# gisbi-kim/lt-mapper

Hardware: AMD Instinct MI355X
Metric: keyframe-pairs/sec (removert+diff) (higher is better)
Workload: dtype f32; 1 GPU; lot-2x500-os1-64-3res; sensor=os1-64

## Files before the change

### include/ltm.h

```cpp
#ifndef LTM_H
#define LTM_H

#include <stddef.h>
#include <stdint.h>

#ifdef __cplusplus
extern "C" {
#endif

#define LTM_ABI_VERSION 1

enum {
    LTM_OK = 0,
    LTM_E_INVALID = -1,
    LTM_E_DEVICE = -2,
    LTM_E_NOMEM = -3,
    LTM_E_UNSUPPORTED = -4
};

typedef struct ltm_ctx ltm_ctx;
typedef uint64_t ltm_cloud;
typedef uint64_t ltm_scanset;
typedef uint64_t ltm_poses;

// ... 36 lines not shown
int ltm_scanset_concat(ltm_ctx*, const ltm_scanset* in, size_t n, ltm_scanset* out);
int ltm_scanset_zip_concat(ltm_ctx*, ltm_scanset a, ltm_scanset b, ltm_scanset c, ltm_scanset* out);
int ltm_scanset_alloc(ltm_ctx*, const uint64_t* offsets, size_t n_kf, ltm_scanset* out);
int ltm_scanset_free(ltm_ctx*, ltm_scanset);

int ltm_buffer_alloc(ltm_ctx*, size_t bytes, void** dev);
int ltm_buffer_free(ltm_ctx*, void* dev);
int ltm_buffer_fill(ltm_ctx*, void* dev, int byte_value, size_t bytes);
int ltm_buffer_copy(ltm_ctx*, void* dst, const void* src, size_t bytes, int kind);

typedef uint64_t ltm_upload;
int ltm_scanset_upload_begin(ltm_ctx*, size_t capacity_points, ltm_upload* up);
int ltm_scanset_upload_chunk(ltm_ctx*, ltm_upload up, const void* pts, size_t stride_bytes, const uint64_t* kf_sizes, size_t n_kf);
int ltm_scanset_upload_end(ltm_ctx*, ltm_upload up, ltm_scanset* out);

typedef struct ltm_fetch ltm_fetch;
int ltm_cloud_fetch_begin(ltm_ctx*, ltm_cloud, ltm_fetch** out);
int ltm_scanset_fetch_begin(ltm_ctx*, ltm_scanset, ltm_fetch** out);
int ltm_fetch_wait(ltm_fetch*, const void** host_xyzi, size_t* n_points, const uint64_t** offsets, size_t* n_kf);
int ltm_fetch_release(ltm_ctx*, ltm_fetch*);
int ltm_cloud_fetch_chunks_begin(ltm_ctx*, ltm_cloud, ltm_fetch** out);
int ltm_scanset_fetch_chunks_begin(ltm_ctx*, ltm_scanset, ltm_fetch** out);
int ltm_fetch_info(ltm_fetch*, size_t* n_points, const uint64_t** offsets, size_t* n_kf);
int ltm_fetch_next_chunk(ltm_fetch*, const void** host_xyzi, size_t* first_point, size_t* n_points, size_t* first_kf, size_t* n_kf);
int ltm_fetch_chunk_done(ltm_fetch*, const void* host_xyzi);

int ltm_poses_create(ltm_ctx*, size_t n_kf, const double* poses, const double* inv_or_null, ltm_poses* out);
int ltm_inverse4x4(const double* m16, double* inv16);
int ltm_poses_free(ltm_ctx*, ltm_poses);


int ltm_preclean(ltm_ctx*, ltm_scanset in, float radius, ltm_scanset* out);

int ltm_merge_to_global(ltm_ctx*, ltm_scanset scans, ltm_poses poses, ltm_cloud* out);

int ltm_voxel_centroid(ltm_ctx*, ltm_cloud in, float leaf, ltm_cloud* out);
int ltm_voxel_centroid_batch(ltm_ctx*, size_t n, const ltm_cloud* in, const float* leaf, ltm_cloud* out);
int ltm_voxel_centroid_shard(ltm_ctx*, ltm_cloud in, float leaf, uint32_t shard, uint32_t n_shards, ltm_cloud* out);
int ltm_cloud_bbox(ltm_ctx*, ltm_cloud in, float mn[3], float mx[3]);
int ltm_voxel_key_histogram(ltm_ctx*, ltm_cloud in, const float mn[3], const float mx[3], float leaf, uint32_t hist[4096]);
int ltm_voxel_key_split(ltm_ctx*, ltm_cloud in, const float mn[3], const float mx[3], float leaf, uint32_t n_parts, const uint32_t* cut_bins, ltm_cloud* parts);
int ltm_voxel_centroid_box(ltm_ctx*, ltm_cloud in, const float mn[3], const float mx[3], float leaf, ltm_cloud* out);
int ltm_voxel_centroid_scanset(ltm_ctx*, ltm_scanset in, float leaf, ltm_scanset* out);

int ltm_voxel_grid_scanset(ltm_ctx*, ltm_scanset in, float leaf, ltm_scanset* out);
typedef struct ltm_vgs ltm_vgs;
int ltm_voxel_grid_scanset_begin(ltm_ctx*, ltm_scanset in, float leaf, ltm_vgs** ticket);
int ltm_voxel_grid_scanset_end(ltm_ctx*, ltm_vgs* ticket, ltm_scanset* out);

int ltm_visibility_vote(ltm_ctx*, ltm_cloud map, ltm_scanset scans, ltm_poses poses, size_t kf_begin, size_t kf_end,
                        float res_alpha, float diff_thres, int mode, uint8_t* labels_dev);
int ltm_scanset_prepare_range_images(ltm_ctx*, ltm_scanset scans, size_t kf_begin, size_t kf_end, const float* res_alphas, size_t n_alphas);
int ltm_partition_by_labels(ltm_ctx*, ltm_cloud map, const uint8_t* labels_dev, ltm_cloud* kept, ltm_cloud* flagged);
int ltm_visibility_partition(ltm_ctx*, ltm_cloud map, ltm_scanset scans, ltm_poses poses, float res_alpha,
                             float diff_thres, int mode, ltm_cloud* kept, ltm_cloud* flagged, uint8_t* host_labels);

int ltm_reproject(ltm_ctx*, ltm_cloud map, ltm_poses poses, size_t kf_begin, size_t kf_end, float res_alpha, ltm_scanset* out);

int ltm_knn_partition(ltm_ctx*, ltm_cloud target, ltm_scanset scans, ltm_poses poses, size_t kf_begin, size_t kf_end,
                      int k, float thr, ltm_scanset* coexist, ltm_scanset* diff);
int ltm_knn_split_cloud(ltm_ctx*, ltm_cloud target, ltm_cloud query, int k, float thr, ltm_cloud* near, ltm_cloud* far);

typedef struct ltm_search ltm_search;
typedef struct ltm_search_result ltm_search_result;
int ltm_search_build(ltm_ctx*, ltm_cloud target, ltm_search** out);
int ltm_search_free(ltm_ctx*, ltm_search*);
int ltm_search_info(ltm_ctx*, ltm_search*, size_t* n_target, size_t* n_finite);
int ltm_knn_search(ltm_ctx*, ltm_search*, ltm_cloud query, int k, int32_t* idx_dev, float* d2_dev);
int ltm_radius_search(ltm_ctx*, ltm_search*, ltm_cloud query, float radius, int max_nn, ltm_search_result** out);
int ltm_search_result_info(ltm_ctx*, ltm_search_result*, size_t* n_query, size_t* total,
                           const uint64_t** offsets_dev, const int32_t** idx_dev, const float** d2_dev);
int ltm_search_result_free(ltm_ctx*, ltm_search_result*);

int ltm_search_estimate_normals(ltm_ctx*, size_t n_idx, ltm_search* const* idx, int k,
                                const float* viewpoints3_or_null );
int ltm_search_normals_info(ltm_ctx*, ltm_search*, int* k , const void** normals_dev );
int ltm_search_normals_download(ltm_ctx*, ltm_search*, float* nxyzc_host );

typedef struct ltm_sc ltm_sc;
typedef struct {
    double lidar_height;
    int    num_ring;
    int    num_sector;
    double max_radius;
    int    num_candidates;
    double search_ratio;
    double dist_thres;
} ltm_sc_params;
void ltm_sc_default_params(ltm_sc_params*);
int  ltm_sc_from_scanset(ltm_ctx*, ltm_scanset, size_t kf_begin, size_t kf_end, const ltm_sc_params*, ltm_sc** out);
int  ltm_sc_from_descriptors(ltm_ctx*, const double* desc_host, size_t n, const ltm_sc_params*, ltm_sc** out);
int  ltm_sc_info(ltm_ctx*, ltm_sc*, size_t* n, int* num_ring, int* num_sector);
int  ltm_sc_download(ltm_ctx*, ltm_sc*, double* desc, float* ring_keys, double* sector_keys);
int  ltm_sc_distance(ltm_ctx*, ltm_sc* a, ltm_sc* b, const int32_t* pairs_host, size_t n_pairs, const ltm_sc_params*, double* dist_host, int32_t* shift_host);
int  ltm_sc_detect(ltm_ctx*, ltm_sc* database, ltm_sc* queries, const ltm_sc_params*, int32_t* loop_id, int32_t* nn_idx, double* min_dist, int32_t* nn_align,
                   float* yaw_diff_rad);
int  ltm_sc_free(ltm_ctx*, ltm_sc*);

typedef struct {
    double max_corr_dist;
    int    max_iterations;
    double transformation_epsilon;
    double euclidean_fitness_epsilon;
} ltm_icp_params;
typedef struct {
    double   T[16];
    double   fitness;
    double   last_mse;
    int32_t  converged;
    int32_t  iterations;
    int32_t  state;
    uint32_t n_corr;
} ltm_icp_result;
void ltm_icp_default_params(ltm_icp_params*);
int  ltm_icp_align(ltm_ctx*, size_t n_pairs, ltm_search* const* targets, const ltm_cloud* sources,
                   const double* init16_or_null , const ltm_icp_params*,
                   ltm_icp_result* results_host, double* trace_host_or_null );
int  ltm_icp_align_scanset(ltm_ctx*, size_t n_pairs, ltm_search* const* targets, ltm_scanset sources, const uint32_t* source_kf ,
                           const double* init16_or_null, const ltm_icp_params*, ltm_icp_result* results_host, double* trace_host_or_null);

int  ltm_icp_align_plane(ltm_ctx*, size_t n_pairs, ltm_search* const* targets, const ltm_cloud* sources,
                         const double* init16_or_null, const ltm_icp_params*, ltm_icp_result* results_host, double* trace_host_or_null);
int  ltm_icp_align_plane_scanset(ltm_ctx*, size_t n_pairs, ltm_search* const* targets, ltm_scanset sources, const uint32_t* source_kf ,
                                 const double* init16_or_null, const ltm_icp_params*, ltm_icp_result* results_host, double* trace_host_or_null);

int ltm_pose6d_to_affine3f(const float* xyzrpy , size_t n, float* affine12 );
int ltm_submaps_assemble(ltm_ctx*, ltm_scanset scans, const float* affine12_host_or_null ,
                         const int32_t* keys_host, size_t n_windows, int search_num, float leaf, int order, ltm_scanset* out);
int ltm_search_build_scanset(ltm_ctx*, ltm_scanset, size_t kf_begin, size_t kf_end, ltm_search** out );

typedef struct ltm_event ltm_event;
int  ltm_lane_create(ltm_ctx* parent, ltm_ctx** lane);
int  ltm_lane_fence(ltm_ctx* done_in, ltm_ctx* before_next_of);
int  ltm_event_record(ltm_ctx*, ltm_event** ev);
int  ltm_event_wait(ltm_ctx*, ltm_event* ev);
void ltm_event_destroy(ltm_event* ev);
int  ltm_cloud_lend(ltm_ctx* from, ltm_cloud h, ltm_ctx* to, ltm_cloud* out);
int  ltm_cloud_give(ltm_ctx* from, ltm_cloud h, ltm_ctx* to, ltm_cloud* out);
int  ltm_scanset_lend(ltm_ctx* from, ltm_scanset h, ltm_ctx* to, ltm_scanset* out);
int  ltm_scanset_give(ltm_ctx* from, ltm_scanset h, ltm_ctx* to, ltm_scanset* out);
int ltm_debug_range_image(ltm_ctx*, ltm_cloud pts, const double* T1, const double* T2, float res_alpha,
                          float* rimg, int32_t* ptidx);
int ltm_debug_viz_images(ltm_ctx*, ltm_cloud map, ltm_scanset scans, ltm_poses poses, size_t kf, float res_alpha, int mode,
                         float range_min, float range_max, float diff_min, float diff_max,
                         uint8_t* scan_bgr, uint8_t* map_bgr, uint8_t* diff_bgr, uint8_t* ptidx_bgr);
int ltm_debug_project(ltm_ctx*, const float* xyz, size_t n, float res_alpha, float* out_az_el_r, int32_t* out_row_col);
void ltm_rimg_size(float vfov, float hfov, float res_alpha, int* rows, int* cols);
int ltm_debug_selfcheck(ltm_ctx*, uint64_t* mismatches3, int* fast_math_enabled);
int ltm_debug_elevation_fit(float vfov_deg, float* c4, double* max_err_rad);
int ltm_debug_pcl_sort_order(const uint32_t* leaf_idx, size_t n, uint32_t* order_out, int use_std_sort, uint32_t* heap_sort_fallbacks );
int ltm_debug_voxel_key_bits(const float* mn3, const float* mx3, float leaf, uint64_t* kept_mask, unsigned* depth, double* frame_min3);
int ltm_debug_proj_launch(float vfov, float hfov, float res_alpha, const double* base2lidar16_or_null, size_t map_points, size_t n_keyframes, int on_device,
                          float* out_f32, uint32_t* out_u32, uint32_t first_block, size_t n_blocks, uint32_t* out_tile, uint32_t* out_kf);
int ltm_debug_cull_check(ltm_ctx*, const float* xyz, size_t n, const double* inv_pose16_or_null, float res_alpha, uint64_t* violations);
int ltm_debug_cull_validation(ltm_ctx*, uint64_t* shapes_checked, uint64_t* shapes_failed);
int ltm_debug_occlusion_stats(ltm_ctx*, uint64_t* pairs, uint64_t* first_shell, uint64_t* projected, int reset);
int ltm_debug_voxel_stats(ltm_ctx*, uint64_t* grids, uint64_t* identity_hits, int reset);
int ltm_debug_knn_stats(ltm_ctx*, uint64_t* queries, uint64_t* undecided, uint64_t* two_phase_calls, uint64_t* unsorted_queue_calls, int reset);
int ltm_debug_sc_paths(int num_ring, int num_sector, int* scatter_in_lds, int* pair_in_lds);
int ltm_debug_cull_stats(ltm_ctx*, uint64_t* survivors, uint64_t* points, int reset);
int ltm_debug_pool_live(ltm_ctx*, uint64_t* live_blocks, uint64_t* live_bytes);

int ltm_profile_enable(ltm_ctx*, int on);
int ltm_profile_reset(ltm_ctx*);
int ltm_profile_read(ltm_ctx*, const char** names, double* ms, uint64_t* launches, double* units, double* bytes, int cap);
int ltm_profile_read_compulsory(ltm_ctx*, double* bytes_c, int cap);

#ifdef __cplusplus
}
#endif
#endif
```

### lt-mapper_amd/capi.py

```python
import ctypes as C
import os

import numpy as np

_HERE = os.path.dirname(os.path.abspath(__file__))
LIB_PATH = os.path.join(_HERE, "libltm_hip.so")

_lib = None

LTM_OK = 0
ERR_NAMES = {0: "LTM_OK", -1: "LTM_E_INVALID", -2: "LTM_E_DEVICE", -3: "LTM_E_NOMEM", -4: "LTM_E_UNSUPPORTED"}


class LtmError(RuntimeError):
    def __init__(self, code, msg):
        super().__init__(f"{ERR_NAMES.get(code, code)}: {msg}")
        self.code = code


class LtmConfig(C.Structure):
    _fields_ = [("vfov", C.c_float), ("hfov", C.c_float), ("lidar2base", C.c_double * 16),
                ("device", C.c_int), ("max_kf_batch", C.c_int)]


class ScParams(C.Structure):
    _fields_ = [("lidar_height", C.c_double), ("num_ring", C.c_int), ("num_sector", C.c_int), ("max_radius", C.c_double),
                ("num_candidates", C.c_int), ("search_ratio", C.c_double), ("dist_thres", C.c_double)]


class IcpParams(C.Structure):
    _fields_ = [("max_corr_dist", C.c_double), ("max_iterations", C.c_int), ("transformation_epsilon", C.c_double),
                ("euclidean_fitness_epsilon", C.c_double)]


ICP_RESULT = np.dtype([("T", np.float64, (4, 4)), ("fitness", np.float64), ("last_mse", np.float64), ("converged", np.int32),
                       ("iterations", np.int32), ("state", np.int32), ("n_corr", np.uint32)], align=True)
ICP_STATES = ("too few correspondences", "iterations", "transform", "absolute mse", "relative mse", "degenerate system")
ICP_METHODS = ("point", "plane")


_vp, _sz, _u64, _i, _f = C.c_void_p, C.c_size_t, C.c_uint64, C.c_int, C.c_float
_pu64 = C.POINTER(C.c_uint64)
_psz = C.POINTER(C.c_size_t)
SIGNATURES = {
    "ltm_abi_version": (_i, []),
    "ltm_create": (_i, [C.POINTER(LtmConfig), C.POINTER(_vp)]),
    "ltm_destroy": (None, [_vp]),
    "ltm_last_error": (C.c_char_p, [_vp]),
    "ltm_synchronize": (_i, [_vp]),
    "ltm_clear_caches": (_i, [_vp]),
    "ltm_stream": (_vp, [_vp]),
    "ltm_cloud_upload": (_i, [_vp, _vp, _sz, _sz, _pu64]),
    "ltm_cloud_from_device": (_i, [_vp, _vp, _sz, _pu64]),
    "ltm_cloud_size": (_i, [_vp, _u64, _psz]),
    "ltm_cloud_download": (_i, [_vp, _u64, _vp, _sz, _sz]),
    "ltm_cloud_device_ptr": (_i, [_vp, _u64, C.POINTER(_vp)]),
    "ltm_cloud_clone": (_i, [_vp, _u64, _pu64]),
    "ltm_cloud_concat": (_i, [_vp, _pu64, _sz, _pu64]),
    "ltm_cloud_transform": (_i, [_vp, _u64, _vp, _vp, _pu64]),
    "ltm_cloud_select": (_i, [_vp, _u64, _vp, _sz, _pu64]),
    "ltm_scanset_keyframe": (_i, [_vp, _u64, _sz, _pu64]),
    "ltm_cloud_free": (_i, [_vp, _u64]),
    "ltm_cloud_alloc": (_i, [_vp, _sz, _pu64]),
    "ltm_scanset_alloc": (_i, [_vp, _pu64, _sz, _pu64]),
    "ltm_scanset_upload_begin": (_i, [_vp, _sz, _pu64]),
    "ltm_scanset_upload_chunk": (_i, [_vp, _u64, _vp, _sz, _pu64, _sz]),
    "ltm_scanset_upload_end": (_i, [_vp, _u64, _pu64]),
    "ltm_cloud_fetch_begin": (_i, [_vp, _u64, C.POINTER(_vp)]),
    "ltm_scanset_fetch_begin": (_i, [_vp, _u64, C.POINTER(_vp)]),
    "ltm_fetch_wait": (_i, [_vp, C.POINTER(_vp), _psz, C.POINTER(_pu64), _psz]),
    "ltm_fetch_release": (_i, [_vp, _vp]),
    "ltm_cloud_fetch_chunks_begin": (_i, [_vp, _u64, C.POINTER(_vp)]),
    "ltm_scanset_fetch_chunks_begin": (_i, [_vp, _u64, C.POINTER(_vp)]),
    "ltm_fetch_info": (_i, [_vp, _psz, C.POINTER(_pu64), _psz]),
    "ltm_fetch_next_chunk": (_i, [_vp, C.POINTER(_vp), _psz, _psz, _psz, _psz]),
    "ltm_fetch_chunk_done": (_i, [_vp, _vp]),
    "ltm_buffer_alloc": (_i, [_vp, _sz, C.POINTER(_vp)]),
    "ltm_buffer_free": (_i, [_vp, _vp]),
    "ltm_buffer_fill": (_i, [_vp, _vp, _i, _sz]),
    "ltm_buffer_copy": (_i, [_vp, _vp, _vp, _sz, _i]),
    "ltm_scanset_upload": (_i, [_vp, _vp, _sz, _pu64, _sz, _pu64]),
    "ltm_scanset_from_device": (_i, [_vp, _vp, _pu64, _sz, _pu64]),
    "ltm_scanset_info": (_i, [_vp, _u64, _psz, _psz]),
    "ltm_scanset_offsets": (_i, [_vp, _u64, _pu64]),
    "ltm_scanset_download": (_i, [_vp, _u64, _vp, _sz, _sz]),
    "ltm_scanset_device_ptr": (_i, [_vp, _u64, C.POINTER(_vp)]),
    "ltm_scanset_as_cloud": (_i, [_vp, _u64, _pu64]),
    "ltm_scanset_concat": (_i, [_vp, _pu64, _sz, _pu64]),
    "ltm_scanset_zip_concat": (_i, [_vp, _u64, _u64, _u64, _pu64]),
    "ltm_scanset_free": (_i, [_vp, _u64]),
    "ltm_poses_create": (_i, [_vp, _sz, _vp, _vp, _pu64]),
    "ltm_poses_free": (_i, [_vp, _u64]),
    "ltm_inverse4x4": (_i, [_vp, _vp]),
    "ltm_preclean": (_i, [_vp, _u64, _f, _pu64]),
    "ltm_merge_to_global": (_i, [_vp, _u64, _u64, _pu64]),
    "ltm_voxel_centroid": (_i, [_vp, _u64, _f, _pu64]),
    "ltm_voxel_centroid_shard": (_i, [_vp, _u64, _f, C.c_uint32, C.c_uint32, _pu64]),
    "ltm_voxel_centroid_batch": (_i, [_vp, _sz, _pu64, C.POINTER(_f), _pu64]),
    "ltm_cloud_bbox": (_i, [_vp, _u64, C.POINTER(_f), C.POINTER(_f)]),
    "ltm_voxel_key_histogram": (_i, [_vp, _u64, C.POINTER(_f), C.POINTER(_f), _f, C.POINTER(C.c_uint32)]),
    "ltm_voxel_key_split": (_i, [_vp, _u64, C.POINTER(_f), C.POINTER(_f), _f, C.c_uint32, C.POINTER(C.c_uint32), _pu64]),
    "ltm_voxel_centroid_box": (_i, [_vp, _u64, C.POINTER(_f), C.POINTER(_f), _f, _pu64]),
    "ltm_voxel_centroid_scanset": (_i, [_vp, _u64, _f, _pu64]),
    "ltm_voxel_grid_scanset": (_i, [_vp, _u64, _f, _pu64]),
    "ltm_voxel_grid_scanset_begin": (_i, [_vp, _u64, _f, C.POINTER(_vp)]),
    "ltm_voxel_grid_scanset_end": (_i, [_vp, _vp, _pu64]),
    "ltm_scanset_prepare_range_images": (_i, [_vp, _u64, _sz, _sz, C.POINTER(_f), _sz]),
    "ltm_visibility_vote": (_i, [_vp, _u64, _u64, _u64, _sz, _sz, _f, _f, _i, _vp]),
    "ltm_partition_by_labels": (_i, [_vp, _u64, _vp, _pu64, _pu64]),
    "ltm_visibility_partition": (_i, [_vp, _u64, _u64, _u64, _f, _f, _i, _pu64, _pu64, _vp]),
    "ltm_lane_create": (_i, [_vp, C.POINTER(_vp)]),
    "ltm_lane_fence": (_i, [_vp, _vp]),
    "ltm_event_record": (_i, [_vp, C.POINTER(_vp)]),
    "ltm_event_wait": (_i, [_vp, _vp]),
    "ltm_event_destroy": (None, [_vp]),
    "ltm_cloud_lend": (_i, [_vp, _u64, _vp, _pu64]),
    "ltm_cloud_give": (_i, [_vp, _u64, _vp, _pu64]),
    "ltm_scanset_lend": (_i, [_vp, _u64, _vp, _pu64]),
    "ltm_scanset_give": (_i, [_vp, _u64, _vp, _pu64]),
    "ltm_reproject": (_i, [_vp, _u64, _u64, _sz, _sz, _f, _pu64]),
    "ltm_knn_partition": (_i, [_vp, _u64, _u64, _u64, _sz, _sz, _i, _f, _pu64, _pu64]),
    "ltm_knn_split_cloud": (_i, [_vp, _u64, _u64, _i, _f, _pu64, _pu64]),
    "ltm_search_build": (_i, [_vp, _u64, C.POINTER(_vp)]),
    "ltm_search_free": (_i, [_vp, _vp]),
    "ltm_search_info": (_i, [_vp, _vp, _psz, _psz]),
    "ltm_knn_search": (_i, [_vp, _vp, _u64, _i, _vp, _vp]),
    "ltm_radius_search": (_i, [_vp, _vp, _u64, _f, _i, C.POINTER(_vp)]),
    "ltm_search_result_info": (_i, [_vp, _vp, _psz, _psz, C.POINTER(_vp), C.POINTER(_vp), C.POINTER(_vp)]),
    "ltm_search_result_free": (_i, [_vp, _vp]),
    "ltm_search_estimate_normals": (_i, [_vp, _sz, C.POINTER(_vp), _i, _vp]),
    "ltm_search_normals_info": (_i, [_vp, _vp, C.POINTER(_i), C.POINTER(_vp)]),
    "ltm_search_normals_download": (_i, [_vp, _vp, _vp]),
    "ltm_sc_default_params": (None, [C.POINTER(ScParams)]),
    "ltm_sc_from_scanset": (_i, [_vp, _u64, _sz, _sz, C.POINTER(ScParams), C.POINTER(_vp)]),
    "ltm_sc_from_descriptors": (_i, [_vp, _vp, _sz, C.POINTER(ScParams), C.POINTER(_vp)]),
    "ltm_sc_info": (_i, [_vp, _vp, _psz, C.POINTER(_i), C.POINTER(_i)]),
    "ltm_sc_download": (_i, [_vp, _vp, _vp, _vp, _vp]),
    "ltm_sc_distance": (_i, [_vp, _vp, _vp, _vp, _sz, C.POINTER(ScParams), _vp, _vp]),
    "ltm_sc_detect": (_i, [_vp, _vp, _vp, C.POINTER(ScParams), _vp, _vp, _vp, _vp, _vp]),
    "ltm_sc_free": (_i, [_vp, _vp]),
    "ltm_icp_default_params": (None, [C.POINTER(IcpParams)]),
    "ltm_icp_align": (_i, [_vp, _sz, C.POINTER(_vp), _pu64, _vp, C.POINTER(IcpParams), _vp, _vp]),
    "ltm_icp_align_scanset": (_i, [_vp, _sz, C.POINTER(_vp), _u64, _vp, _vp, C.POINTER(IcpParams), _vp, _vp]),
    "ltm_icp_align_plane": (_i, [_vp, _sz, C.POINTER(_vp), _pu64, _vp, C.POINTER(IcpParams), _vp, _vp]),
    "ltm_icp_align_plane_scanset": (_i, [_vp, _sz, C.POINTER(_vp), _u64, _vp, _vp, C.POINTER(IcpParams), _vp, _vp]),
    "ltm_pose6d_to_affine3f": (_i, [_vp, _sz, _vp]),
    "ltm_submaps_assemble": (_i, [_vp, _u64, _vp, _vp, _sz, _i, _f, _i, _pu64]),
    "ltm_search_build_scanset": (_i, [_vp, _u64, _sz, _sz, C.POINTER(_vp)]),
    "ltm_debug_pool_live": (_i, [_vp, _pu64, _pu64]),
    "ltm_debug_range_image": (_i, [_vp, _u64, _vp, _vp, _f, _vp, _vp]),
    "ltm_debug_viz_images": (_i, [_vp, _u64, _u64, _u64, _sz, _f, _i, _f, _f, _f, _f, _vp, _vp, _vp, _vp]),
    "ltm_debug_project": (_i, [_vp, _vp, _sz, _f, _vp, _vp]),
    "ltm_debug_elevation_fit": (_i, [_f, C.POINTER(_f), C.POINTER(C.c_double)]),
    "ltm_debug_pcl_sort_order": (_i, [C.POINTER(C.c_uint32), C.c_size_t, C.POINTER(C.c_uint32), _i, C.POINTER(C.c_uint32)]),
    "ltm_debug_voxel_key_bits": (_i, [C.POINTER(_f), C.POINTER(_f), _f, _pu64, C.POINTER(C.c_uint), C.POINTER(C.c_double)]),
    "ltm_debug_selfcheck": (_i, [_vp, _pu64, C.POINTER(_i)]),
    "ltm_debug_cull_check": (_i, [_vp, _vp, _sz, _vp, _f, _pu64]),
    "ltm_debug_cull_stats": (_i, [_vp, _pu64, _pu64, _i]),
    "ltm_debug_proj_launch": (_i, [_f, _f, _f, _vp, _sz, _sz, _i, _vp, _vp, C.c_uint32, _sz, _vp, _vp]),
    "ltm_debug_cull_validation": (_i, [_vp, _pu64, _pu64]),
    "ltm_debug_occlusion_stats": (_i, [_vp, _pu64, _pu64, _pu64, _i]),
    "ltm_debug_voxel_stats": (_i, [_vp, _pu64, _pu64, _i]),
    "ltm_debug_knn_stats": (_i, [_vp, _pu64, _pu64, _pu64, _pu64, _i]),
    "ltm_debug_sc_paths": (_i, [_i, _i, C.POINTER(_i), C.POINTER(_i)]),
    "ltm_rimg_size": (None, [_f, _f, _f, C.POINTER(_i), C.POINTER(_i)]),
    "ltm_profile_enable": (_i, [_vp, _i]),
    "ltm_profile_reset": (_i, [_vp]),
    "ltm_profile_read_compulsory": (_i, [_vp, C.POINTER(C.c_double), _i]),
    "ltm_profile_read": (_i, [_vp, C.POINTER(C.c_char_p), C.POINTER(C.c_double), _pu64, C.POINTER(C.c_double),
                              C.POINTER(C.c_double), _i]),
}


def load_library(path=None):
    global _lib
    if _lib is not None and path is None:
        return _lib
    p = path or LIB_PATH
    try:
        import torch
    except Exception:
        pass
    if not os.path.exists(p):
        raise FileNotFoundError(
            f"{p} not found: build it with `make hip` (or __graft_entry__.build()). There is no CPU fallback.")
    lib = C.CDLL(p)
    for name, (res, args) in SIGNATURES.items():
        fn = getattr(lib, name)
        fn.restype = res
        fn.argtypes = args
    if path is None:
        _lib = lib
    return lib


def voxel_key_bits(mn, mx, leaf):
    a = (_f * 3)(*[float(v) for v in mn]); b = (_f * 3)(*[float(v) for v in mx])
    mask, depth, fmin = _u64(), C.c_uint(), (C.c_double * 3)()
    n = load_library().ltm_debug_voxel_key_bits(a, b, float(leaf), C.byref(mask), C.byref(depth), fmin)
    if n < 0:
        raise ValueError("unsupported box / leaf")
    return n, mask.value, depth.value, np.array(list(fmin))


PROJ_LAUNCH_F32 = ("half_v", "half_h", "inv_v", "inv_h", "frows", "fcols", "row_max", "col_max", "row_scale", "col_scale", "row_bias", "col_bias",
                   "certain_lim", "rmin2", "eps", "el_tclamp")
PROJ_LAUNCH_U32 = ("rows", "cols", "npx", "steep_clamps", "packable", "n_tiles", "n_tg", "tg_magic", "tg_shift", "grid", "el_fit", "fast")


def proj_launch(vfov, hfov, alpha, base2lidar=None, map_points=0, n_keyframes=1, on_device=False, first_block=0, n_blocks=0):
    f = np.zeros(len(PROJ_LAUNCH_F32), dtype=np.float32)
    u = np.zeros(len(PROJ_LAUNCH_U32), dtype=np.uint32)
    tile = np.zeros(max(n_blocks, 1), dtype=np.uint32)
    kf = np.zeros(max(n_blocks, 1), dtype=np.uint32)
    b2l = None if base2lidar is None else _mat16(base2lidar)
    rc = load_library().ltm_debug_proj_launch(float(vfov), float(hfov), float(alpha), None if b2l is None else b2l.ctypes.data, int(map_points),
                                              int(n_keyframes), int(bool(on_device)), f.ctypes.data, u.ctypes.data, int(first_block), int(n_blocks),
                                              tile.ctypes.data, kf.ctypes.data)
    if rc != 0:
        raise LtmError(rc, "ltm_debug_proj_launch")
    return dict(zip(PROJ_LAUNCH_F32, f)), {k: int(v) for k, v in zip(PROJ_LAUNCH_U32, u)}, tile[:n_blocks], kf[:n_blocks]


def inverse4x4(m):
    a = np.ascontiguousarray(m, dtype=np.float64).reshape(16)
    out = np.empty(16, dtype=np.float64)
    if load_library().ltm_inverse4x4(a.ctypes.data, out.ctypes.data) != 0:
        raise ValueError("singular or non-finite matrix")
    return out.reshape(4, 4)


def pose6d_to_affine3f(xyzrpy):
    a = np.ascontiguousarray(xyzrpy, dtype=np.float32).reshape(-1, 6)
    out = np.empty((a.shape[0], 3, 4), dtype=np.float32)
    if a.shape[0] and load_library().ltm_pose6d_to_affine3f(a.ctypes.data, a.shape[0], out.ctypes.data) != 0:
        raise ValueError("ltm_pose6d_to_affine3f failed")
    return out


ORDERS = {"input": 0, "pcl": 1}


def _np_pts(a):
    a = np.ascontiguousarray(a, dtype=np.float32)
    if a.ndim != 2 or a.shape[1] != 4:
        a = a.reshape(-1, 4)
    return a


def _mat16(m):
    m = np.ascontiguousarray(m, dtype=np.float64).reshape(-1)
    assert m.size == 16
    return m


class Context:

    def __init__(self, vfov=50.0, hfov=360.0, lidar2base=None, device=0, max_kf_batch=0):
        self.lib = load_library()
        cfg = LtmConfig()
        cfg.vfov, cfg.hfov, cfg.device, cfg.max_kf_batch = vfov, hfov, device, max_kf_batch
        l2b = _mat16(np.eye(4) if lidar2base is None else lidar2base)
        for i in range(16):
            cfg.lidar2base[i] = l2b[i]
        self.vfov, self.hfov, self.device = float(vfov), float(hfov), int(device)
        h = _vp()
        rc = self.lib.ltm_create(C.byref(cfg), C.byref(h))
        if rc != LTM_OK:
            raise LtmError(rc, "ltm_create failed (no usable gfx950 device?)")
        self.h = h

    def lane(self):
        other = Context.__new__(Context)
        other.lib, other.vfov, other.hfov, other.device = self.lib, self.vfov, self.hfov, self.device
        h = _vp()
        rc = self.lib.ltm_lane_create(self.h, C.byref(h))
        if rc != LTM_OK:
            raise LtmError(rc, "ltm_lane_create failed")
        other.h = h
        return other

    def _pass(self, obj, to, give):
        kind = "cloud" if isinstance(obj, Cloud) else "scanset"
        out = _u64()
        self._ck(getattr(self.lib, f"ltm_{kind}_{'give' if give else 'lend'}")(self.h, obj.h, to.h, C.byref(out)))
        new = (Cloud if kind == "cloud" else ScanSet)(to, out.value)
        if give:
            obj.h = 0
        else:
            new._lender = obj
        return new

    def lend(self, obj, to):
        return self._pass(obj, to, False)

    def give(self, obj, to):
        return self._pass(obj, to, True)

    def fence(self, before_next_of):
        self._ck(self.lib.ltm_lane_fence(self.h, before_next_of.h))

    def event_record(self):
        ev = _vp()
        self._ck(self.lib.ltm_event_record(self.h, C.byref(ev)))
        return Event(self.lib, ev)

    def event_wait(self, ev):
        self._ck(self.lib.ltm_event_wait(self.h, ev.h))

    def close(self):
        if getattr(self, "h", None):
            self.lib.ltm_destroy(self.h)
            self.h = None

    def __del__(self):
        try:
            self.close()
        except Exception:
            pass

    def _ck(self, rc):
        if rc != LTM_OK:
            raise LtmError(rc, self.lib.ltm_last_error(self.h).decode())

    def upload(self, pts):
        a = _np_pts(pts)
        out = _u64()
        self._ck(self.lib.ltm_cloud_upload(self.h, a.ctypes.data, a.shape[0], 16, C.byref(out)))
        return Cloud(self, out.value)

    def cloud_from_device(self, dev_ptr, n):
        out = _u64()
        self._ck(self.lib.ltm_cloud_from_device(self.h, dev_ptr, n, C.byref(out)))
        return Cloud(self, out.value)

    def transform(self, cloud, T1=None, T2=None):
        t1 = None if T1 is None else np.ascontiguousarray(T1, dtype=np.float64).reshape(16)
        t2 = None if T2 is None else np.ascontiguousarray(T2, dtype=np.float64).reshape(16)
        out = _u64()
        self._ck(self.lib.ltm_cloud_transform(self.h, cloud.h, None if t1 is None else t1.ctypes.data, None if t2 is None else t2.ctypes.data, C.byref(out)))
        return Cloud(self, out.value)

    def select(self, cloud, idx):
        a = np.ascontiguousarray(idx, dtype=np.int32)
        out = _u64()
        self._ck(self.lib.ltm_cloud_select(self.h, cloud.h, a.ctypes.data, a.size, C.byref(out)))
        return Cloud(self, out.value)

    def scan_of_keyframe(self, scans, kf):
        out = _u64()
        self._ck(self.lib.ltm_scanset_keyframe(self.h, scans.h, kf, C.byref(out)))
        return Cloud(self, out.value)

    def concat(self, clouds):
        arr = (_u64 * len(clouds))(*[c.h for c in clouds])
        out = _u64()
        self._ck(self.lib.ltm_cloud_concat(self.h, arr, len(clouds), C.byref(out)))
        return Cloud(self, out.value)

    def upload_scans(self, pts, offsets):
        a = _np_pts(pts)
        off = np.ascontiguousarray(offsets, dtype=np.uint64)
        out = _u64()
        self._ck(self.lib.ltm_scanset_upload(self.h, a.ctypes.data, 16, off.ctypes.data_as(_pu64), off.size - 1, C.byref(out)))
        return ScanSet(self, out.value)

    def scans_from_device(self, dev_ptr, offsets):
        off = np.ascontiguousarray(offsets, dtype=np.uint64)
        out = _u64()
        self._ck(self.lib.ltm_scanset_from_device(self.h, dev_ptr, off.ctypes.data_as(_pu64), off.size - 1, C.byref(out)))
        return ScanSet(self, out.value)

    def concat_scansets(self, sets):
        arr = (_u64 * len(sets))(*[s.h for s in sets])
# ... 698 lines not shown
```

### lt-mapper_amd/csrc/ltm_api_core.cpp

```cpp
#include "ltm_internal.h"

namespace ltm_detail {

bool inverse4x4(const double* m, double* inv)
{
    double A[2][2], B[2][2], C[2][2], D[2][2];
    for (int r = 0; r < 2; ++r)
        for (int k = 0; k < 2; ++k) {
            A[r][k] = m[4 * k + r]; B[r][k] = m[4 * (k + 2) + r];
            C[r][k] = m[4 * k + r + 2]; D[r][k] = m[4 * (k + 2) + r + 2];
        }
    const double dA = A[0][0] * A[1][1] - A[0][1] * A[1][0], dB = B[0][0] * B[1][1] - B[0][1] * B[1][0];
    const double dC = C[0][0] * C[1][1] - C[0][1] * C[1][0], dD = D[0][0] * D[1][1] - D[0][1] * D[1][0];
    double AB[2][2], DC[2][2];
    for (int j = 0; j < 2; ++j) {
        AB[0][j] = B[0][j] * A[1][1] - B[1][j] * A[0][1]; AB[1][j] = B[1][j] * A[0][0] - B[0][j] * A[1][0];
        DC[0][j] = C[0][j] * D[1][1] - C[1][j] * D[0][1]; DC[1][j] = C[1][j] * D[0][0] - C[0][j] * D[1][0];
    }
    const double tr = (AB[0][0] * DC[0][0] + AB[1][0] * DC[0][1]) + (AB[0][1] * DC[1][0] + AB[1][1] * DC[1][1]);
    double iA[2][2], iB[2][2], iC[2][2], iD[2][2];
    for (int i = 0; i < 2; ++i)
        for (int j = 0; j < 2; ++j) {
            iD[i][j] = D[i][j] * dA - (AB[0][j] * C[i][0] + AB[1][j] * C[i][1]);
            iA[i][j] = A[i][j] * dD - (DC[0][j] * B[i][0] + DC[1][j] * B[i][1]);
// ... 41 lines not shown
        c_lo[r] = cr - (double)out[9 + r];
        for (int k = 0; k < 3; ++k) out[3 * r + k] = (float)T[4 * r + k];
    }
    for (int r = 0; r < 3; ++r)
        out[12 + r] = (float)-((double)out[3 * r] * c_lo[0] + (double)out[3 * r + 1] * c_lo[1] + (double)out[3 * r + 2] * c_lo[2]);
    double gmin = 1e300;
    for (int a2 = 0; a2 < 3; ++a2) {
        double diag = 0, off = 0;
        for (int b2 = 0; b2 < 3; ++b2) {
            double g2 = 0;
            for (int r = 0; r < 3; ++r) g2 += T[4 * r + a2] * T[4 * r + b2];
            if (a2 == b2) diag = g2; else off += std::fabs(g2);
        }
        gmin = std::min(gmin, diag - off);
    }
    double smin = gmin > 0.25 ? std::sqrt(gmin) * (1.0 - 1e-6) : 0.0;
    double gmax = 0.0;
    for (int a2 = 0; a2 < 3; ++a2) {
        double row = 0;
        for (int b2 = 0; b2 < 3; ++b2) {
            double g2 = 0;
            for (int r = 0; r < 3; ++r) g2 += T[4 * r + a2] * T[4 * r + b2];
            row += std::fabs(g2);
        }
        gmax = std::max(gmax, row);
    }
    if (!(std::sqrt(gmax) * (1.0 + 1e-6) < 1.001)) smin = std::min(smin, 0.99);
    out[15] = smin > 0.5 ? (float)std::nextafter((float)smin, 0.0f) : 1.0e-30f;
}

static double fit_elevation_poly(double tmax, float c_out[4])
{
    const int N = 4000;
    std::vector<double> t(N), y(N), w(N, 1.0 / N), B(4 * (size_t)N);
    for (int i = 0; i < N; ++i) {
        t[i] = tmax * (i + 1) / N;
        y[i] = std::atan(t[i]);
        const double u = (t[i] / tmax) * (t[i] / tmax);
        double b = t[i];
        for (int k = 0; k < 4; ++k) { B[4 * (size_t)i + k] = b; b *= u; }
    }
    double c[4] = {1.0, 0.0, 0.0, 0.0};
    for (int it = 0; it < 200; ++it) {
        double M[4][5] = {};
        for (int i = 0; i < N; ++i)
            for (int r = 0; r < 4; ++r) {
                const double wb = w[i] * B[4 * (size_t)i + r];
                for (int k = 0; k < 4; ++k) M[r][k] += wb * B[4 * (size_t)i + k];
                M[r][4] += wb * y[i];
            }
        for (int col = 0; col < 4; ++col) {
            int piv = col;
            for (int r = col + 1; r < 4; ++r) if (std::fabs(M[r][col]) > std::fabs(M[piv][col])) piv = r;
            for (int k = 0; k < 5; ++k) std::swap(M[col][k], M[piv][k]);
            if (M[col][col] == 0.0) return 1.0;
            for (int r = 0; r < 4; ++r) {
                if (r == col) continue;
                const double f = M[r][col] / M[col][col];
                for (int k = col; k < 5; ++k) M[r][k] -= f * M[col][k];
            }
        }
        for (int k = 0; k < 4; ++k) c[k] = M[k][4] / M[k][k];
        double sum = 0.0;
        for (int i = 0; i < N; ++i) {
            double p = 0.0;
            for (int k = 0; k < 4; ++k) p += c[k] * B[4 * (size_t)i + k];
            w[i] *= std::fabs(p - y[i]);
            sum += w[i];
        }
        if (!(sum > 0.0)) break;
        for (int i = 0; i < N; ++i) w[i] /= sum;
    }
    double scale = 1.0;
    for (int k = 0; k < 4; ++k) { c_out[k] = (float)(c[k] * scale); scale /= tmax * tmax; }
    double worst = 0.0;
    const int G = 200000;
    for (int i = 0; i <= G; ++i) {
        const float tf = (float)(tmax * i / G), uu = tf * tf;
        const float pf = tf * std::fmaf(std::fmaf(std::fmaf(c_out[3], uu, c_out[2]), uu, c_out[1]), uu, c_out[0]);
        worst = std::max(worst, std::fabs((double)pf - std::atan((double)tf)));
    }
    return worst;
}

int elevation_fit_for(float vfov, float c4[4], double* err)
{
    c4[0] = 1.0f; c4[1] = c4[2] = c4[3] = 0.0f;
    *err = 0.0;
    if (!(vfov > 0.0f) || 0.5 * (double)vfov + 2.0 > 45.0) return 0;
    *err = fit_elevation_poly(std::tan((0.5 * (double)vfov + 2.0) * (3.14159265358979323846 / 180.0)), c4);
    return *err <= 1.0e-6 ? 1 : 0;
}

void pack_from_host(const void* src, size_t n, size_t stride, std::vector<float>& out)
{
    out.resize(n * 4);
    const unsigned char* s = static_cast<const unsigned char*>(src);
    const size_t ioff = (stride >= 32) ? 16 : 12;
    for (size_t i = 0; i < n; ++i) {
        memcpy(&out[4 * i], s + i * stride, 12);
        memcpy(&out[4 * i + 3], s + i * stride + ioff, 4);
    }
}
void unpack_to_host(const float* packed, size_t n, size_t stride, void* dst)
{
    unsigned char* d = static_cast<unsigned char*>(dst);
    const float one = 1.0f;
    for (size_t i = 0; i < n; ++i) {
        unsigned char* p = d + i * stride;
        if (stride >= 32) {
            memset(p, 0, 32);
            memcpy(p, &packed[4 * i], 12); memcpy(p + 12, &one, 4); memcpy(p + 16, &packed[4 * i + 3], 4);
        } else {
            memcpy(p, &packed[4 * i], 16);
        }
    }
}



}

extern "C" {

int ltm_abi_version(void) { return LTM_ABI_VERSION; }

int ltm_create(const ltm_config* cfg, ltm_ctx** out)
{
    if (!cfg || !out) return LTM_E_INVALID;
    *out = nullptr;
    int ndev = 0;
    if (hipGetDeviceCount(&ndev) != hipSuccess || ndev <= 0) return LTM_E_DEVICE;
    if (cfg->device < 0 || cfg->device >= ndev) return LTM_E_INVALID;
    ltm_ctx* c = new (std::nothrow) ltm_ctx();
    if (!c) return LTM_E_NOMEM;
    c->cfg = *cfg;
    c->device = cfg->device;
    if (cfg->max_kf_batch > 0) c->kf_batch = (size_t)cfg->max_kf_batch;
    double b2l[16];
    if (!(cfg->vfov > 0.0f) || !(cfg->hfov > 0.0f) || !inverse4x4(cfg->lidar2base, b2l)) { delete c; return LTM_E_INVALID; }
    c->l2b_identity = mat_is_identity(cfg->lidar2base);
    if (c->l2b_identity) memcpy(b2l, cfg->lidar2base, sizeof b2l);
    c->b2l_identity = mat_is_identity(b2l);
    c->L2B = to34(cfg->lidar2base); c->B2L = to34(b2l);
    if (hipSetDevice(c->device) != hipSuccess || hipStreamCreateWithFlags(&c->stream, hipStreamNonBlocking) != hipSuccess) {
        delete c;
        return LTM_E_DEVICE;
    }
    c->pool.stream = c->stream;
    auto env_int = [](const char* name, int dflt) { const char* v = getenv(name); return v ? atoi(v) : dflt; };
    c->kopts.map_kernel_variant = env_int("LTM_MAP_KERNEL", 2);
    c->kopts.vote_cull = env_int("LTM_VOTE_CULL", 1);
    c->kopts.tile_cull = env_int("LTM_TILE_CULL", 1);
    c->kopts.stats_blockmin = env_int("LTM_STATS_BLOCKMIN", 0);
    {
        unsigned long long* d = nullptr;
        bool ok = hipMalloc(&d, 3 * sizeof(unsigned long long)) == hipSuccess && hipMemsetAsync(d, 0, 24, c->stream) == hipSuccess &&
                  selfcheck_fast_math(cfg->vfov, cfg->hfov, d, c->stream) == hipSuccess &&
                  hipMemcpyAsync(c->selfcheck, d, 24, hipMemcpyDeviceToHost, c->stream) == hipSuccess &&
                  hipStreamSynchronize(c->stream) == hipSuccess;
        if (d) (void)hipFree(d);
        if (!ok) { (void)hipStreamDestroy(c->stream); delete c; return LTM_E_DEVICE; }
        c->fast_math = (c->selfcheck[0] == 0 && c->selfcheck[1] == 0 && c->selfcheck[2] == 0) ? 1 : 0;
        if (const char* v = getenv("LTM_KNN_FAST")) c->knn_two_phase = atoi(v);
        if (const char* v = getenv("LTM_VOXEL_KEYBITS")) c->voxel_key_compress = atoi(v);
        if (const char* v = getenv("LTM_VOXEL_FUSED_TAIL")) c->voxel_fused_tail = atoi(v);
        if (const char* v = getenv("LTM_VOXEL_IDENTITY")) c->voxel_identity = atoi(v);
        if (const char* v = getenv("LTM_OCCLUSION")) c->occlusion_cull = atoi(v);
        if (getenv("LTM_OCCLUSION_STATS")) c->occlusion_stats_on = 1;
        if (const char* v = getenv("LTM_OCCLUSION_MIN_PAIRS")) c->occlusion_min_pairs = (size_t)atoll(v);
        if (const char* v = getenv("LTM_OCCLUSION_RNEAR")) {
            const float r = (float)atof(v);
            c->occlusion_r_near = std::isfinite(r) ? std::max(1.0f, r) : 60.0f;
        }
        if (const char* v = getenv("LTM_KNN_STATS")) c->knn_stats_on = atoi(v);
        if (const char* v = getenv("LTM_CULL_SELFCHECK")) c->cull_selfcheck = atoi(v);
        if (const char* v = getenv("LTM_CULL_EPS_SCALE")) c->cull_eps_scale = (float)atof(v);
        if (const char* v = getenv("LTM_CULL_EPS_FLOOR")) c->cull_eps_floor = (float)atof(v);
        c->el_fit = elevation_fit_for(c->cfg.vfov, c->el_c, &c->el_fit_err);
        if (const char* v = getenv("LTM_HEAVY_CHAIN")) c->heavy_chain_on = atoi(v);
        if (const char* v = getenv("LTM_HEAVY_MIN_BLOCKS")) c->heavy_min_blocks = (size_t)atoll(v);
    }
    c->heavy = std::make_shared<HeavyChain>();
    *out = c;
    return LTM_OK;
}

void ltm_destroy(ltm_ctx* c)
{
    if (!c) return;
    (void)hipSetDevice(c->device);
    (void)hipStreamSynchronize(c->stream);
    vgs_release_all(c);
    search_release_all(c);
    sc_release_all(c);
    for (Pending& p : c->pending) { (void)hipEventDestroy(p.a); (void)hipEventDestroy(p.b); }
    for (hipEvent_t e : c->event_pool) (void)hipEventDestroy(e);
    if (c->copy_stream) { (void)hipStreamSynchronize(c->copy_stream); (void)hipStreamDestroy(c->copy_stream); }
    for (auto& kv : c->uploads) { for (int b = 0; b < 2; ++b) if (kv.second.ev[b]) (void)hipEventDestroy(kv.second.ev[b]); c->pool.free(kv.second.d); }
    for (PinnedBlock& b : c->pinned) (void)hipHostFree(b.p);
    if (c->scratch_pinned) (void)hipHostFree(c->scratch_pinned);
    if (c->live_counts) (void)hipFree(c->live_counts);
    if (getenv("LTM_OCCLUSION_STATS") && c->occl_pairs)
        fprintf(stderr, "[ltm] occlusion cull of the exact-image kernel: %llu (tile, keyframe) pairs, %.2f %% in the first shell, %.2f %% projected in all, %.2f %% dropped\n",
                (unsigned long long)c->occl_pairs, 100.0 * c->occl_near / c->occl_pairs, 100.0 * c->occl_far_live / c->occl_pairs,
                100.0 * (c->occl_pairs - c->occl_far_live) / c->occl_pairs);
    if (getenv("LTM_OCCLUSION_STATS") && c->occl_quarters)
        fprintf(stderr, "[ltm] occlusion cull, second look: %llu 1024-point quarters in the pairs left alive, %.2f %% of them projected\n",
                (unsigned long long)c->occl_quarters, 100.0 * c->occl_quarters_live / c->occl_quarters);
    if (c->knn_stats_on && c->knn_queries)
        fprintf(stderr, "[ltm] kNN two-phase: %llu of %llu scan queries left undecided by the bucket test (%.2f %%)\n", (unsigned long long)c->knn_undecided,
                (unsigned long long)c->knn_queries, 100.0 * (double)c->knn_undecided / (double)c->knn_queries);
    if (getenv("LTM_POOL_STATS"))
        fprintf(stderr, "[ltm] device pool: %zu hipMalloc calls, %.1f MB held, %.1f ms inside hipMalloc; pinned host blocks: %zu, %.1f MB, %.1f ms inside hipHostMalloc\n",
                c->pool.n_malloc, c->pool.bytes_total / 1048576.0, 1e3 * c->pool.malloc_s, c->pinned.size(), c->pinned_bytes / 1048576.0, 1e3 * c->pinned_s);
    c->pool.release_all();
    (void)hipStreamDestroy(c->stream);
    delete c;
}

const char* ltm_last_error(const ltm_ctx* c) { return c ? c->err.c_str() : "null context"; }

int ltm_synchronize(ltm_ctx* c) { return guarded(c, [&] { sync(c); }); }

int ltm_clear_caches(ltm_ctx* c) { return guarded(c, [&] { sync(c); scan_cache_drop(c, 0); }); }

void* ltm_stream(ltm_ctx* c) { return c ? (void*)c->stream : nullptr; }

void ltm_rimg_size(float vfov, float hfov, float alpha, int* rows, int* cols)
{
    if (rows) *rows = (int)roundf(vfov * alpha);
    if (cols) *cols = (int)roundf(hfov * alpha);
}

int ltm_cloud_upload(ltm_ctx* c, const void* pts, size_t n, size_t stride, ltm_cloud* out)
{
    return guarded(c, [&] {
        LTM_REQUIRE(out && (pts || n == 0), "null argument");
        LTM_REQUIRE(stride == 16 || stride >= 32 || n == 0, "stride must be 16 (packed) or >= 32 (pcl::PointXYZI)");
        float4* d;
        const ltm_cloud h = alloc_cloud(c, n, &d);
        if (n) {
            if (stride == 16) h2d(c, d, pts, n * 16);
            else { std::vector<float> tmp; pack_from_host(pts, n, stride, tmp); h2d(c, d, tmp.data(), n * 16); }
        }
        *out = h;
    });
}

int ltm_cloud_from_device(ltm_ctx* c, const void* dev, size_t n, ltm_cloud* out)
{
    return guarded(c, [&] {
        LTM_REQUIRE(out && (dev || n == 0), "null argument");
        float4* d;
        const ltm_cloud h = alloc_cloud(c, n, &d);
        d2d(c, d, dev, n * 16);
        sync(c);
        *out = h;
    });
}

int ltm_cloud_size(ltm_ctx* c, ltm_cloud h, size_t* n)
{
    return guarded(c, [&] { LTM_REQUIRE(n, "null argument"); *n = get_cloud(c, h).n; });
}

int ltm_cloud_download(ltm_ctx* c, ltm_cloud h, void* dst, size_t cap, size_t stride)
{
    return guarded(c, [&] {
        const Cloud& cl = get_cloud(c, h);
        LTM_REQUIRE(dst || cl.n == 0, "null destination");
        LTM_REQUIRE(cap >= cl.n, "destination too small");
        LTM_REQUIRE(stride == 16 || stride >= 32, "stride must be 16 or >= 32");
        if (!cl.n) return;
        if (stride == 16) d2h(c, dst, cl.d, cl.n * 16);
        else { std::vector<float> tmp(cl.n * 4); d2h(c, tmp.data(), cl.d, cl.n * 16); unpack_to_host(tmp.data(), cl.n, stride, dst); }
    });
}

int ltm_cloud_device_ptr(ltm_ctx* c, ltm_cloud h, const void** p)
{
    return guarded(c, [&] { LTM_REQUIRE(p, "null argument"); *p = get_cloud(c, h).d; });
}

int ltm_cloud_clone(ltm_ctx* c, ltm_cloud h, ltm_cloud* out)
{
    return guarded(c, [&] {
        LTM_REQUIRE(out, "null argument");
        const Cloud src = get_cloud(c, h);
        float4* d;
        const ltm_cloud nh = alloc_cloud(c, src.n, &d);
        d2d(c, d, src.d, src.n * 16);
        inherit_frame(c, nh, src);
        *out = nh;
    });
}

int ltm_cloud_concat(ltm_ctx* c, const ltm_cloud* in, size_t n, ltm_cloud* out)
{
    return guarded(c, [&] {
        LTM_REQUIRE(out && (in || n == 0), "null argument");
        size_t tot = 0;
        for (size_t i = 0; i < n; ++i) tot += get_cloud(c, in[i]).n;
        float4* d;
        const ltm_cloud h = alloc_cloud(c, tot, &d);
        size_t at = 0;
// ... 768 lines not shown
```

### lt-mapper_amd/csrc/ltm_api_vote.cpp

```cpp
#include "ltm_internal.h"

namespace ltm_detail {

static Geom geom_from(float vfov, float hfov, float alpha, int fast_math, int el_fit, const float* el_c, float cull_eps_scale, float cull_eps_floor)
{
    Geom g;
    g.vfov = vfov; g.hfov = hfov;
    g.rows = (int)roundf(vfov * alpha);
    g.cols = (int)roundf(hfov * alpha);
    g.fast = fast_math;
    const float ppd = std::max((float)g.rows / g.vfov, (float)g.cols / g.hfov);
    const float scale = cull_eps_scale > 0.0f ? cull_eps_scale : (el_fit ? 3.0e-4f : 6.0e-4f);
    g.cull_eps_px = std::max(cull_eps_floor, scale * ppd);
    g.el_fit = el_fit;
    for (int i = 0; i < 4; ++i) g.el_c[i] = el_c[i];
    const double out_deg = std::min(2.0, (double)g.vfov / std::max(g.rows, 1));
    g.el_tclamp = (float)std::tan((0.5 * (double)g.vfov + out_deg) * (3.14159265358979323846 / 180.0));
    return g;
}
Geom geom_for(const ltm_ctx* c, float alpha)
{
    return geom_from(c->cfg.vfov, c->cfg.hfov, alpha, c->fast_math, c->el_fit, c->el_c, c->cull_eps_scale, c->cull_eps_floor);
}

// ... 111 lines not shown
        }
        ProfScope p(c, "vote_scan", (double)npts * n, (double)npts * 16 * n + px_all * 4, (double)npts * 16 + px_all * 4);
        for (int j = 0; j < n; ++j) {
            LTM_HIP(fill_u32(imgs[j], kNoPointBits, nb * (size_t)rows[j] * cols[j], c->stream));
            LTM_HIP(hipMemsetAsync(smax[j], 0, nb * sizeof(uint32_t), c->stream));
        }
        LTM_HIP(scan_range_images_multi(ss.d, ss.off_dev, kb, nb, npts, longest, todo[at], n, rows, cols, imgs, smax, c->stream));
    }
}

bool cull_geometry_ok(ltm_ctx* c, const Geom& g, const Poses& ps, size_t kf)
{
    if (!c->cull_selfcheck) return true;
    const std::pair<int, int> key(g.rows, g.cols);
    auto it = c->cull_geom_ok.find(key);
    if (it != c->cull_geom_ok.end()) return it->second;
    const size_t n = (size_t)1 << 20;
    DevBuf pts(c, n * 12), bad(c, 8);
    LTM_HIP(hipMemsetAsync(bad.p, 0, 8, c->stream));
    LTM_HIP(cull_probe_points(g, n, nullptr, pts.as<float>(), c->stream));
    LTM_HIP(cull_check(pts.as<float>(), n, nullptr, &c->B2L, c->b2l_identity, nullptr, g, bad.as<unsigned long long>(), c->stream));
    if (ps.approx_dev && kf < ps.n) {
        const HostMat34 pose = to34(&ps.pose[16 * kf]), inv = to34(&ps.inv[16 * kf]);
        LTM_HIP(cull_probe_points(g, n, &pose, pts.as<float>(), c->stream));
        LTM_HIP(cull_check(pts.as<float>(), n, &inv, &c->B2L, c->b2l_identity, ps.approx_dev + 16 * kf, g, bad.as<unsigned long long>(), c->stream));
    }
    unsigned long long v = 0;
    d2h(c, &v, bad.p, 8);
    const bool ok = v == 0;
    ++c->cull_geoms_checked;
    if (!ok) {
        ++c->cull_geoms_failed;
        fprintf(stderr, "[ltm] the bounded-error projection left its validated bounds for the %d x %d range image (%llu of %zu probe points): exact kernels for this shape\n",
                g.rows, g.cols, v, 2 * n);
    }
    c->cull_geom_ok[key] = ok;
    return ok;
}

void exact_map_images(ltm_ctx* c, const Cloud& map, const Poses& ps, size_t kb, size_t nb, const Geom& g, uint64_t* img)
{
    if (!map.n || !nb) return;
    const size_t n_tiles = (map.n + 4095) / 4096, n_pairs = n_tiles * nb;
    KernelOpts ko = c->kopts;
    if (ko.map_kernel_variant >= 2 && ps.approx_dev && !cull_geometry_ok(c, g, ps, kb)) ko.map_kernel_variant = 1;
    const bool occl = c->occlusion_cull && ko.map_kernel_variant >= 2 && ps.approx_dev && n_pairs >= c->occlusion_min_pairs && n_pairs < 0xffffffffull;
    if (!occl) {
        HeavyScope hs(c, n_pairs);
        LTM_HIP(map_range_images(map.d, map.n, ps.inv_dev, ps.approx_dev, kb, nb, c->B2L, c->b2l_identity, g, img, hs.stream(), ko));
        hs.done();
        return;
    }
    const size_t rbs = (size_t)g.rows, cbs = ((size_t)g.cols + 7) / 8;
    const size_t tbytes = scan_temp_bytes(n_pairs);
    const size_t dwords = (rbs + 31) / 32;
    const bool subtiles = c->occlusion_subtile != 0;
    const size_t need = n_tiles * 24 + n_pairs * (1 + 1 + 4 + 4) + 64 + nb * rbs * cbs * 4 + nb * dwords * 4 + tbytes + (subtiles ? n_tiles * 96 + n_pairs + 64 : 0) + 12 * 256;
    if (c->occl_scratch_bytes < need) {
        if (c->occl_scratch) { sync(c); c->pool.free(c->occl_scratch); c->occl_scratch = nullptr; c->occl_scratch_bytes = 0; }
        c->occl_scratch = c->pool.alloc(need + need / 4);
        c->occl_scratch_bytes = need + need / 4;
    }
    char* base = static_cast<char*>(c->occl_scratch);
    auto carve = [&](size_t bytes) { char* p = base; base += (bytes + 255) & ~(size_t)255; return p; };
    float* tb = reinterpret_cast<float*>(carve(n_tiles * 24));
    uint8_t* done = reinterpret_cast<uint8_t*>(carve(n_pairs));
    uint8_t* flags = reinterpret_cast<uint8_t*>(carve(n_pairs));
    uint32_t* pos = reinterpret_cast<uint32_t*>(carve(n_pairs * 4));
    uint32_t* list = reinterpret_cast<uint32_t*>(carve(n_pairs * 4));
    uint32_t* count = reinterpret_cast<uint32_t*>(carve(64));
    uint32_t* cmax = reinterpret_cast<uint32_t*>(carve(nb * rbs * cbs * 4));
    uint32_t* dirty = reinterpret_cast<uint32_t*>(carve(nb * dwords * 4));
    void* temp = carve(tbytes);
    float* tbq = subtiles ? reinterpret_cast<float*>(carve(n_tiles * 96)) : nullptr;
    uint8_t* submask = subtiles ? reinterpret_cast<uint8_t*>(carve(n_pairs)) : nullptr;
    unsigned long long* sub_stats = subtiles ? reinterpret_cast<unsigned long long*>(carve(64)) : nullptr;
    LTM_HIP(tile_bounds(map.d, map.n, tb, c->stream));
    if (subtiles) {
        LTM_HIP(subtile_bounds(map.d, map.n, tbq, c->stream));
        LTM_HIP(hipMemsetAsync(sub_stats, 0, 16, c->stream));
    }
    LTM_HIP(hipMemsetAsync(done, 0, n_pairs, c->stream));
    if (dirty) {
        LTM_HIP(hipMemsetAsync(dirty, 0, nb * dwords * 4, c->stream));
        LTM_HIP(fill_u32(cmax, 0x461c4000u, nb * rbs * cbs, c->stream));
    }
    float r_lo = 0.0f, r_hi = c->occlusion_r_near;
    size_t n_done = 0, n_proj = 0;
    for (int shell = 0; shell < 12; ++shell) {
        const bool last = shell == 11 || r_hi > 1.0e4f;
        if (last) r_hi = 3.0e38f;
        LTM_HIP(occlusion_shell_pairs(ps.approx_dev, kb, nb, tb, n_tiles, g, r_lo, r_hi, img, shell > 0, cmax, done, flags, pos, list, count, temp, tbytes, c->stream, dirty,
                                      tbq, submask, c->occlusion_stats_on ? sub_stats : nullptr));
        uint32_t n_live = 0;
        d2h(c, &n_live, count, 4);
        {
            HeavyScope hs(c, n_live);
            LTM_HIP(map_range_images_pairs(map.d, map.n, ps.inv_dev, ps.approx_dev, kb, nb, c->B2L, c->b2l_identity, g, img, list, n_live, hs.stream(), ko, submask));
            hs.done();
        }
        n_proj += n_live;
        if (shell == 0) c->occl_near += n_live;
        if (last) break;
        r_lo = r_hi; r_hi *= 2.0f;
    }
    (void)n_done;
    if (subtiles && c->occlusion_stats_on) {
        unsigned long long st[2] = {0, 0};
        d2h(c, st, sub_stats, 16);
        c->occl_quarters += st[0]; c->occl_quarters_live += st[1];
    }
    c->occl_pairs += n_pairs; c->occl_far_live += n_proj;
}

void do_vote(ltm_ctx* c, const Cloud& map, uint64_t ss_handle, const ScanSet& ss, const Poses& ps, size_t kf_begin, size_t kf_end, float alpha, float thr,
             int mode, uint8_t* labels_dev)
{
    LTM_REQUIRE(ss.nkf() == ps.n, "scan set and poses have different keyframe counts");
    LTM_REQUIRE(kf_begin <= kf_end && kf_end <= ps.n, "keyframe range out of bounds");
    LTM_REQUIRE(mode == 0 || mode == 1, "mode must be 0 (scan-map) or 1 (map-scan)");
    LTM_REQUIRE(map.n < 0xffffffffull, "map too large for 32-bit point indices");
    if (kf_begin == kf_end || map.n == 0) return;
    const Geom g = geom_for(c, alpha);
    LTM_REQUIRE(g.rows > 0 && g.cols > 0, "empty range image");
    const size_t npx = (size_t)g.rows * g.cols;
    const size_t KB = std::min(c->kf_batch, kf_end - kf_begin);
    DevBuf map_img(c, KB * npx * sizeof(uint64_t));
    const size_t n_tiles = (map.n + 4095) / 4096;
    DevBuf tb(c, n_tiles * 6 * sizeof(float));
    if (mode == 0) LTM_HIP(tile_bounds(map.d, map.n, tb.as<float>(), c->stream));
    for (size_t kb = kf_begin; kb < kf_end; kb += KB) {
        const size_t nb = std::min(KB, kf_end - kb);
        const uint32_t* smax = nullptr;
        const float* qbound = nullptr;
        const bool cull = mode == 0 && (c->kopts.vote_cull != 0) && ps.approx_dev && cull_geometry_ok(c, g, ps, kb);
        const uint32_t* scan_img = scan_images(c, ss_handle, ss, kb, nb, g, &smax, cull ? thr : -1.0f, &qbound);
        {
            ProfScope p(c, "vote_fill", (double)(nb * npx), (double)(nb * npx * 8));
            LTM_HIP(fill_u64(map_img.as<uint64_t>(), (uint64_t)kNoPointBits << 32, nb * npx, c->stream));
        }
        {
            double pts = (double)map.n * nb, bytes = 16.0 * pts + (double)nb * 8.0 * npx, bytes_c = 16.0 * map.n + (double)nb * (cull ? 12.0 : 8.0) * npx;
            const bool count_live = cull && c->prof_on && (c->kopts.tile_cull != 0) && smax && c->pending_live.size() < (size_t)kLiveSlots;
            if (count_live) {
                if (!c->live_counts) LTM_HIP(hipMalloc(reinterpret_cast<void**>(&c->live_counts), sizeof(unsigned long long) * kLiveSlots));
                const int slot = (int)c->pending_live.size();
                LTM_HIP(hipMemsetAsync(c->live_counts + slot, 0, sizeof(unsigned long long), c->stream));
                LTM_HIP(count_live_tiles(ps.approx_dev, kb, nb, tb.as<float>(), n_tiles, smax, thr, c->live_counts + slot, c->stream));
                c->pending_live.push_back(PendingLive{prof_class(c, "vote_map_cull"), slot, pts, (double)nb * 8.0 * npx, (double)map.n, (double)nb * 12.0 * npx});
                pts = 0.0; bytes = 0.0; bytes_c = 0.0;
            }
            ProfScope p(c, cull ? "vote_map_cull" : "vote_map_exact", pts, bytes, bytes_c);
            if (cull) {
                HeavyScope hs(c, n_tiles * nb);
                LTM_HIP(vote_map_range_images(map.d, map.n, ps.inv_dev, ps.approx_dev, kb, nb, c->B2L, c->b2l_identity, g, qbound, tb.as<float>(), smax, thr, mode,
                                              map_img.as<uint64_t>(), hs.stream(), c->kopts));
                hs.done();
            } else exact_map_images(c, map, ps, kb, nb, g, map_img.as<uint64_t>());
        }
        {
            ProfScope p(c, "vote_compare", (double)(nb * npx), (double)(nb * npx) * 12 + (double)nb * map.n / 8.0);
            LTM_HIP(compare_and_flag(scan_img, map_img.as<uint64_t>(), nb * npx, thr, mode, labels_dev, c->stream));
        }
    }
}

void do_partition(ltm_ctx* c, const Cloud& map, const uint8_t* labels, ltm_cloud* kept, ltm_cloud* flagged)
{
    const size_t n = map.n;
    if (n == 0) {
        float4* d;
        if (kept) *kept = alloc_cloud(c, 0, &d);
        if (flagged) *flagged = alloc_cloud(c, 0, &d);
        return;
    }
    DevBuf pos(c, n * sizeof(uint32_t));
    ProfScope p(c, "partition", (double)n, (double)n * (16 + 1 + 4 + 4 + 16));
    const size_t nf = count_flags(c, labels, n, pos);
    float4 *dk = nullptr, *df = nullptr;
    ltm_cloud hk = 0, hf = 0;
    if (kept) hk = alloc_cloud(c, n - nf, &dk);
    if (flagged) hf = alloc_cloud(c, nf, &df);
    LTM_HIP(partition_scatter(map.d, labels, pos.as<uint32_t>(), n, dk, df, c->stream));
    if (kept) { *kept = hk; inherit_frame(c, hk, map); }
    if (flagged) { *flagged = hf; inherit_frame(c, hf, map); }
}


}

extern "C" {

int ltm_scanset_prepare_range_images(ltm_ctx* c, ltm_scanset hs, size_t kf_begin, size_t kf_end, const float* alphas, size_t n_alphas)
{
    return guarded(c, [&] {
        LTM_REQUIRE(alphas || n_alphas == 0, "null argument");
        const ScanSet& ss = get_ss(c, hs);
        LTM_REQUIRE(kf_begin <= kf_end && kf_end <= ss.nkf(), "keyframe range out of bounds");
        if (kf_begin == kf_end || n_alphas == 0) return;
        std::vector<Geom> geoms;
        for (size_t i = 0; i < n_alphas; ++i) geoms.push_back(geom_for(c, alphas[i]));
        const size_t KB = std::min(c->kf_batch, kf_end - kf_begin);
        for (size_t kb = kf_begin; kb < kf_end; kb += KB) scan_images_prepare(c, hs, ss, kb, std::min(KB, kf_end - kb), geoms);
    });
}

int ltm_visibility_vote(ltm_ctx* c, ltm_cloud hmap, ltm_scanset hs, ltm_poses hp, size_t kf_begin, size_t kf_end, float alpha,
                        float thr, int mode, uint8_t* labels_dev)
{
    return guarded(c, [&] {
        LTM_REQUIRE(labels_dev, "null labels buffer");
        do_vote(c, get_cloud(c, hmap), hs, get_ss(c, hs), get_poses(c, hp), kf_begin, kf_end, alpha, thr, mode, labels_dev);
        sync(c);
    });
}

int ltm_partition_by_labels(ltm_ctx* c, ltm_cloud hmap, const uint8_t* labels_dev, ltm_cloud* kept, ltm_cloud* flagged)
{
    return guarded(c, [&] {
        LTM_REQUIRE(labels_dev || get_cloud(c, hmap).n == 0, "null labels buffer");
        const Cloud map = get_cloud(c, hmap);
        do_partition(c, map, labels_dev, kept, flagged);
        sync(c);
    });
}

int ltm_visibility_partition(ltm_ctx* c, ltm_cloud hmap, ltm_scanset hs, ltm_poses hp, float alpha, float thr, int mode,
                             ltm_cloud* kept, ltm_cloud* flagged, uint8_t* host_labels)
{
    return guarded(c, [&] {
        const Cloud map = get_cloud(c, hmap);
        const Poses& p = get_poses(c, hp);
        DevBuf labels(c, std::max<size_t>(map.n, 1));
        LTM_HIP(hipMemsetAsync(labels.p, 0, std::max<size_t>(map.n, 1), c->stream));
        do_vote(c, map, hs, get_ss(c, hs), p, 0, p.n, alpha, thr, mode, labels.as<uint8_t>());
        if (host_labels) d2h(c, host_labels, labels.p, map.n);
        do_partition(c, map, labels.as<uint8_t>(), kept, flagged);
    });
}

int ltm_reproject(ltm_ctx* c, ltm_cloud hmap, ltm_poses hp, size_t kf_begin, size_t kf_end, float alpha, ltm_scanset* out)
{
    return guarded(c, [&] {
        LTM_REQUIRE(out, "null argument");
        const Cloud map = get_cloud(c, hmap);
        const Poses& p = get_poses(c, hp);
        LTM_REQUIRE(kf_begin <= kf_end && kf_end <= p.n, "keyframe range out of bounds");
        LTM_REQUIRE(map.n < 0xffffffffull, "map too large for 32-bit point indices");
        const Geom g = geom_for(c, alpha);
        LTM_REQUIRE(g.rows > 0 && g.cols > 0, "empty range image");
        const size_t npx = (size_t)g.rows * g.cols;
        const size_t nk = kf_end - kf_begin;
        std::vector<uint64_t> off(nk + 1, 0);
        struct Piece { float4* d; size_t n; };
        std::vector<Piece> pieces;
        if (nk && map.n) {
            const size_t KB = std::min(c->kf_batch, nk);
            DevBuf img(c, KB * npx * 8), pos(c, KB * npx * 4);
            const size_t tb = scan_temp_bytes(KB * npx);
            DevBuf temp(c, tb), bout(c, (KB + 1) * 4);
            for (size_t kb = kf_begin; kb < kf_end; kb += KB) {
                const size_t nb = std::min(KB, kf_end - kb);
                LTM_HIP(fill_u64(img.as<uint64_t>(), (uint64_t)kNoPointBits << 32, nb * npx, c->stream));
                {
                    ProfScope ps(c, "reproject_map", (double)map.n * nb, (double)nb * (16.0 * map.n + 8.0 * npx), 16.0 * map.n + (double)nb * 8.0 * npx);
                    exact_map_images(c, map, p, kb, nb, g, img.as<uint64_t>());
                }
                ProfScope ps(c, "reproject_gather", (double)(nb * npx), (double)(nb * npx) * 12);
                LTM_HIP(exclusive_scan_img_valid(img.as<uint64_t>(), pos.as<uint32_t>(), nb * npx, temp.p, tb, c->stream));
                LTM_HIP(image_bounds(pos.as<uint32_t>(), img.as<uint64_t>(), npx, nb, bout.as<uint32_t>(), c->stream));
                std::vector<uint32_t> b(nb + 1);
                d2h(c, b.data(), bout.p, (nb + 1) * 4);
                const size_t total = b[nb];
                const uint64_t base = off[kb - kf_begin];
                for (size_t j = 1; j <= nb; ++j) off[kb - kf_begin + j] = base + b[j];
                float4* d = reinterpret_cast<float4*>(c->pool.alloc(std::max<size_t>(total, 1) * 16));
                LTM_HIP(reproject_gather(img.as<uint64_t>(), pos.as<uint32_t>(), npx, nb, map.d, p.inv_dev, kb, c->B2L, c->b2l_identity, d, c->stream));
                pieces.push_back(Piece{d, total});
            }
        }
        float4* d = nullptr;
        if (pieces.size() == 1) d = pieces[0].d;
        else {
            d = reinterpret_cast<float4*>(c->pool.alloc(std::max<size_t>(off[nk], 1) * 16));
            size_t at = 0;
            for (Piece& pc : pieces) { d2d(c, d + at, pc.d, pc.n * 16); at += pc.n; }
            sync(c);
            for (Piece& pc : pieces) c->pool.free(pc.d);
        }
        *out = new_scanset(c, d, std::move(off));
    });
}

int ltm_debug_range_image(ltm_ctx* c, ltm_cloud h, const double* T1, const double* T2, float alpha, float* rimg, int32_t* ptidx)
{
    return guarded(c, [&] {
        LTM_REQUIRE(rimg, "null argument");
        const Cloud cl = get_cloud(c, h);
        const Geom g = geom_for(c, alpha);
        const size_t npx = (size_t)g.rows * g.cols;
        DevBuf img(c, npx * 8), r(c, npx * 4), ix(c, npx * 4);
        LTM_HIP(fill_u64(img.as<uint64_t>(), (uint64_t)kNoPointBits << 32, npx, c->stream));
        HostMat34 a, b;
        if (T1) a = to34(T1);
        if (T2) b = to34(T2);
        LTM_HIP(single_range_image(cl.d, cl.n, T1 ? &a : nullptr, T2 ? &b : nullptr, g, img.as<uint64_t>(), c->stream));
        LTM_HIP(decode_image(img.as<uint64_t>(), npx, r.as<float>(), ix.as<int32_t>(), c->stream));
        d2h(c, rimg, r.p, npx * 4);
        if (ptidx) d2h(c, ptidx, ix.p, npx * 4);
    });
}

static void jet_lut_bgr(uint8_t* lut)
{
    for (int i = 0; i < 256; ++i) {
        const double x = (double)i / 255.0;
        const double bgr[3] = {std::min(4.0 * x + 0.5, 2.5 - 4.0 * x), std::min(4.0 * x - 0.5, 3.5 - 4.0 * x), std::min(4.0 * x - 1.5, 4.5 - 4.0 * x)};
        for (int ch = 0; ch < 3; ++ch) {
            const float sample = (float)std::min(1.0, std::max(0.0, bgr[ch]));
            lut[3 * i + ch] = (uint8_t)std::min(255l, std::max(0l, std::lrint((double)(sample * 255.0f))));
        }
    }
}

int ltm_debug_viz_images(ltm_ctx* c, ltm_cloud hmap, ltm_scanset hscans, ltm_poses hposes, size_t kf, float alpha, int mode,
                         float range_min, float range_max, float diff_min, float diff_max,
                         uint8_t* scan_bgr, uint8_t* map_bgr, uint8_t* diff_bgr, uint8_t* ptidx_bgr)
{
    return guarded(c, [&] {
        LTM_REQUIRE(mode == 0 || mode == 1, "mode must be 0 (scan-map) or 1 (map-scan)");
        LTM_REQUIRE(range_max != range_min && diff_max != diff_min, "empty colour axis");
        const Cloud map = get_cloud(c, hmap);
        const ScanSet& ss = get_ss(c, hscans);
        const Poses& ps = get_poses(c, hposes);
        LTM_REQUIRE(ss.nkf() == ps.n && kf < ps.n, "keyframe out of range");
        LTM_REQUIRE(map.n < 0x7fffffffull, "map too large for an int32 index image");
        const Geom g = geom_for(c, alpha);
        const size_t npx = (size_t)g.rows * g.cols;
        const uint32_t* smax = nullptr;
        const uint32_t* scan_img = scan_images(c, hscans, ss, kf, 1, g, &smax);
        DevBuf img(c, npx * 8), mr(c, npx * 4), mi(c, npx * 4), df(c, npx * 4), out(c, npx * 3), lutd(c, 768);
        LTM_HIP(fill_u64(img.as<uint64_t>(), (uint64_t)kNoPointBits << 32, npx, c->stream));
        if (map.n)
            LTM_HIP(map_range_images(map.d, map.n, ps.inv_dev, ps.approx_dev, kf, 1, c->B2L, c->b2l_identity, g, img.as<uint64_t>(), c->stream, c->kopts));
        LTM_HIP(decode_image(img.as<uint64_t>(), npx, mr.as<float>(), mi.as<int32_t>(), c->stream));
        uint8_t lut[768];
        jet_lut_bgr(lut);
        h2d(c, lutd.p, lut, sizeof lut);
        auto axis = [](float lo, float hi, double* a, double* b) {
            const double inv = 1.0 / (double)(float)(hi - lo);
            *a = 255.0 * inv; *b = -((double)lo * 255.0) * inv;
        };
        double a, b;
        auto emit_f32 = [&](const float* src, uint8_t* host) {
            if (!host) return;
            LTM_HIP(viz_colormap_f32(src, npx, (float)a, (float)b, lutd.as<uint8_t>(), out.as<uint8_t>(), c->stream));
            d2h(c, host, out.p, npx * 3);
        };
        axis(range_min, range_max, &a, &b);
        emit_f32(reinterpret_cast<const float*>(scan_img), scan_bgr);
        emit_f32(mr.as<float>(), map_bgr);
        if (diff_bgr) {
            LTM_HIP(viz_diff(scan_img, mr.as<float>(), npx, mode, df.as<float>(), c->stream));
            axis(diff_min, diff_max, &a, &b);
            emit_f32(df.as<float>(), diff_bgr);
        }
        if (ptidx_bgr) {
            LTM_REQUIRE(map.n > 0, "index image of an empty map has no colour axis");
            axis(0.0f, (float)map.n, &a, &b);
            LTM_HIP(viz_colormap_i32(mi.as<int32_t>(), npx, a, b, lutd.as<uint8_t>(), out.as<uint8_t>(), c->stream));
            d2h(c, ptidx_bgr, out.p, npx * 3);
        }
    });
}

int ltm_debug_project(ltm_ctx* c, const float* xyz, size_t n, float alpha, float* sph, int32_t* rc)
{
    return guarded(c, [&] {
        LTM_REQUIRE((xyz && sph && rc) || n == 0, "null argument");
        if (!n) return;
        const Geom g = geom_for(c, alpha);
        DevBuf in(c, n * 12), o1(c, n * 12), o2(c, n * 8);
        h2d(c, in.p, xyz, n * 12);
        LTM_HIP(debug_project(in.as<float>(), n, g, o1.as<float>(), o2.as<int32_t>(), c->stream));
        d2h(c, sph, o1.p, n * 12);
        d2h(c, rc, o2.p, n * 8);
    });
}

int ltm_debug_cull_check(ltm_ctx* c, const float* xyz, size_t n, const double* inv_pose16, float alpha, uint64_t* violations)
{
    return guarded(c, [&] {
        LTM_REQUIRE((xyz && violations) || n == 0, "null argument");
        if (violations) *violations = 0;
        if (!n) return;
        const Geom g = geom_for(c, alpha);
        DevBuf in(c, n * 12), bad(c, 8), apd(c, 64);
        h2d(c, in.p, xyz, n * 12);
        LTM_HIP(hipMemsetAsync(bad.p, 0, 8, c->stream));
        HostMat34 T{};
        if (inv_pose16) {
            float ap[16];
            double b2l16[16] = {0};
            memcpy(b2l16, c->B2L.m, 12 * sizeof(double)); b2l16[15] = 1.0;
            approx_pose(b2l16, inv_pose16, ap);
            h2d(c, apd.p, ap, 64);
            T = to34(inv_pose16);
        }
        LTM_HIP(cull_check(in.as<float>(), n, inv_pose16 ? &T : nullptr, &c->B2L, c->b2l_identity, apd.as<float>(), g, bad.as<unsigned long long>(), c->stream));
        unsigned long long v = 0;
        d2h(c, &v, bad.p, 8);
        *violations = v;
    });
}

int ltm_debug_cull_validation(ltm_ctx* c, uint64_t* shapes_checked, uint64_t* shapes_failed)
{
    return guarded(c, [&] { if (shapes_checked) *shapes_checked = c->cull_geoms_checked; if (shapes_failed) *shapes_failed = c->cull_geoms_failed; });
}

int ltm_debug_proj_launch(float vfov, float hfov, float alpha, const double* base2lidar16, size_t map_points, size_t n_keyframes, int on_device,
                          float* out_f32, uint32_t* out_u32, uint32_t first_block, size_t n_blocks, uint32_t* out_tile, uint32_t* out_kf)
{
    if (!(vfov > 0.0f) || !(hfov > 0.0f) || !(alpha > 0.0f) || !out_f32 || !out_u32 || (n_blocks && (!out_tile || !out_kf))) return LTM_E_INVALID;
    if (map_points >= 0xffffffffull || n_keyframes >= 0xffffffffull) return LTM_E_INVALID;
    float el_c[4];
    double err = 0.0;
    const int el_fit = elevation_fit_for(vfov, el_c, &err);
    const Geom g = geom_from(vfov, hfov, alpha, 0, el_fit, el_c, 0.0f, 1.0e-3f);
    if (g.rows <= 0 || g.cols <= 0) return LTM_E_INVALID;
    HostMat34 b2l{};
    b2l.m[0] = b2l.m[5] = b2l.m[10] = 1.0;
    int ident = 1;
    if (base2lidar16) { b2l = to34(base2lidar16); ident = mat_is_identity(base2lidar16) ? 1 : 0; }
    if (proj_launch_debug(g, b2l, ident, map_points, n_keyframes, on_device, out_f32, out_u32) != hipSuccess) return LTM_E_DEVICE;
    if (n_blocks) proj_launch_blocks(map_points, n_keyframes, first_block, n_blocks, out_tile, out_kf);
    return LTM_OK;
}

int ltm_debug_cull_stats(ltm_ctx* c, uint64_t* survivors, uint64_t* points, int reset)
{
    return guarded(c, [&] {
        unsigned long long v[2] = {0, 0};
        LTM_HIP(cull_stats(v, reset, c->stream, c->kopts.stats_blockmin));
        if (survivors) *survivors = v[0];
        if (points) *points = v[1];
    });
}

int ltm_debug_occlusion_stats(ltm_ctx* c, uint64_t* pairs, uint64_t* first_shell, uint64_t* projected, int reset)
{
    return guarded(c, [&] {
        if (pairs) *pairs = c->occl_pairs;
        if (first_shell) *first_shell = c->occl_near;
        if (projected) *projected = c->occl_far_live;
        if (reset) { c->occl_pairs = 0; c->occl_near = 0; c->occl_far_live = 0; }
    });
}

}
```

### lt-mapper_amd/csrc/ltm_k_projection.hip

```cpp
#include "ltm_kernels_common.h"
#include <rocprim/device/device_scan.hpp>
#include <rocprim/iterator/transform_iterator.hpp>

namespace ltm {

__global__ void k_fill_u32(uint32_t* p, uint32_t v, size_t n)
{
    size_t i = (size_t)blockIdx.x * blockDim.x + threadIdx.x;
    const size_t stride = (size_t)gridDim.x * blockDim.x;
    for (; i < n; i += stride) p[i] = v;
}
__global__ void k_fill_u64(uint64_t* p, uint64_t v, size_t n)
{
    size_t i = (size_t)blockIdx.x * blockDim.x + threadIdx.x;
    const size_t stride = (size_t)gridDim.x * blockDim.x;
    for (; i < n; i += stride) p[i] = v;
}
hipError_t fill_u32(uint32_t* p, uint32_t v, size_t n, hipStream_t s)
{
    if (!n) return hipSuccess;
    k_fill_u32<<<dim3((unsigned)std::min<size_t>(grid_for(n), 8192)), dim3(kBlock), 0, s>>>(p, v, n);
    return hipGetLastError();
}
hipError_t fill_u64(uint64_t* p, uint64_t v, size_t n, hipStream_t s)
// ... 267 lines not shown
__device__ __forceinline__ float3 xform_approx(const float* __restrict__ ap, float4 p4, bool& ok)
{
    const float dx = p4.x - ap[9], dy = p4.y - ap[10], dz = p4.z - ap[11];
    ok = ap[15] != 0.0f;
    float3 o;
    o.x = __builtin_fmaf(ap[2], dz, __builtin_fmaf(ap[1], dy, __builtin_fmaf(ap[0], dx, ap[12])));
    o.y = __builtin_fmaf(ap[5], dz, __builtin_fmaf(ap[4], dy, __builtin_fmaf(ap[3], dx, ap[13])));
    o.z = __builtin_fmaf(ap[8], dz, __builtin_fmaf(ap[7], dy, __builtin_fmaf(ap[6], dx, ap[14])));
    return o;
}

template <bool EL3 = false>
__device__ __forceinline__ CullCand cull_candidates(const ProjLaunch& pl, float3 p)
{
    const RimgGeom& g = pl.g;
    CullCand cc;
    const float xy2 = __builtin_fmaf(p.x, p.x, p.y * p.y);
    cc.r2 = __builtin_fmaf(p.z, p.z, xy2);
    const float inv_rxy = __builtin_amdgcn_rsqf(xy2);
    const float t_el = fabsf(p.z) * inv_rxy;
    const float ax = fabsf(p.x), ay = fabsf(p.y);
    const float az_oct = asin_octant_approx(fminf(ax, ay) * inv_rxy);
    float el_abs;
    if (EL3) {
        const float t = fminf(t_el, g.el_tclamp), u = t * t;
        el_abs = t * __builtin_fmaf(__builtin_fmaf(__builtin_fmaf(g.el_c3, u, g.el_c2), u, g.el_c1), u, g.el_c0);
    } else {
        el_abs = atan_unit_approx(fminf(t_el, 1.0f));
    }
    const float el = __builtin_copysignf(el_abs, p.z);
    float az = (ay > ax) ? (1.57079632679f - az_oct) : az_oct;
    az = (p.x < 0.0f) ? (3.14159265359f - az) : az;
    az = __builtin_copysignf(az, p.y);
    cc.rowh = __builtin_fmaf(el, -pl.row_scale, pl.row_bias);
    cc.colh = __builtin_fmaf(az, pl.col_scale, pl.col_bias);
    const bool certain = fmaxf(__builtin_amdgcn_fractf(cc.rowh), __builtin_amdgcn_fractf(cc.colh)) < pl.certain_lim;
    cc.unusual = (fabsf(p.y) <= __builtin_fmaf(-1.0e-6f, p.x, 1.0e-18f)) | (cc.r2 > 6.4e7f);
    if (!EL3) cc.unusual |= !pl.steep_clamps & (t_el > 1.0f);
    cc.multi = !certain;
    cc.rb = (int)__builtin_amdgcn_fmed3f(cc.rowh, 0.0f, g.row_max);
    cc.cb = (int)__builtin_amdgcn_fmed3f(cc.colh, 0.0f, g.col_max);
    cc.r0 = cc.r1 = cc.rb; cc.c0 = cc.c1 = cc.cb;
    return cc;
}

__device__ __forceinline__ float cull_r_lo(float r2) { return __builtin_amdgcn_sqrtf(r2) * (1.0f - 1.5e-6f); }

__device__ __forceinline__ void cull_expand(const ProjLaunch& pl, CullCand& cc)
{
    const RimgGeom& g = pl.g;
    const float rfl = floorf(cc.rowh), cfl = floorf(cc.colh);
    const float rfr = cc.rowh - rfl, cfr = cc.colh - cfl;
    const int rc = (int)rfl, ccn = (int)cfl;
    const int rmax = g.rows - 1, cmax = g.cols - 1;
    const float lim = pl.certain_lim;
    cc.r0 = min(max(rc, 0), rmax);
    cc.r1 = min(max(rc + (rfr >= lim ? 1 : 0), 0), rmax);
    cc.c0 = min(max(ccn, 0), cmax);
    cc.c1 = min(max(ccn + (cfr >= lim ? 1 : 0), 0), cmax);
}


__device__ unsigned long long g_cull_stats[4];

static constexpr int kCullQueue = 2048;

template <int ROWS, int COLS>
__device__ __forceinline__ int table_claim(uint32_t* __restrict__ tags, int row, int col, uint32_t px)
{
    const int slot = ((row & (ROWS - 1)) * COLS) | (col & (COLS - 1));
    uint32_t t = tags[slot];
    if (t == kEmptyTag) {
        const uint32_t old = atomicCAS(&tags[slot], kEmptyTag, px);
        t = (old == kEmptyTag) ? px : old;
    }
    return (t == px) ? slot : -1;
}

template <bool B2L_IDENTITY, int SLOTS_R, int SLOTS_C>
__device__ __forceinline__ void exact_insert(const float4* __restrict__ map, uint32_t i, const Mat34& Tinv, const HostMat34& b2l_h, const RimgGeom& g,
                                             uint64_t* __restrict__ vals, uint32_t* __restrict__ tags, uint64_t* __restrict__ imgk)
{
    const float4 p4 = map[i];
    float3 p = xform(Tinv, make_float3(p4.x, p4.y, p4.z));
    if (B2L_IDENTITY) p = xform_identity(p); else p = xform(to_dev(b2l_h), p);
    const Sph s = cart2sph(p.x, p.y, p.z);
    int row, col;
    pixel_row_col(g, s.az, s.el, row, col);
    const uint32_t px = (uint32_t)(row * g.cols + col);
    const uint64_t v = ((uint64_t)f2u(s.r) << 32) | (uint64_t)i;
    const int slot = table_claim<SLOTS_R, SLOTS_C>(tags, row, col, px);
    if (slot >= 0) { if (v < vals[slot]) atomicMin(reinterpret_cast<unsigned long long*>(&vals[slot]), (unsigned long long)v); }
    else img_min_u64(imgk + px, v);
}

template <bool B2L_IDENTITY>
__device__ __forceinline__ uint32_t exact_range_bits(const float4 p4, const Mat34& Tinv, const HostMat34& b2l_h)
{
    float3 p = xform(Tinv, make_float3(p4.x, p4.y, p4.z));
    if (B2L_IDENTITY) p = xform_identity(p); else p = xform(to_dev(b2l_h), p);
    const float xy = p.x * p.x + p.y * p.y;
    return f2u(__builtin_sqrtf(xy + p.z * p.z));
}

__device__ __forceinline__ bool tile_out_of_reach(const float* __restrict__ ap, const float* __restrict__ tb, float smax, float thr)
{
    float d2 = 0.0f, far2 = 0.0f;
#pragma unroll
    for (int d = 0; d < 3; ++d) {
        const float c = ap[9 + d];
        const float lo = tb[d] - c, hi = c - tb[3 + d];
        const float e = fmaxf(fmaxf(lo, hi), 0.0f);
        const float f = fmaxf(fabsf(lo), fabsf(hi));
        d2 = __builtin_fmaf(e, e, d2);
        far2 = __builtin_fmaf(f, f, far2);
    }
    const float smin = ap[15];
    const float reach = fmaxf(smax - thr, 0.0f) + 1.0e-2f + smax * 1.0e-3f;
    return smin > 0.5f && far2 < 8.0e7f && d2 * smin * smin * 0.996f > reach * reach;
}

__global__ void __launch_bounds__(kBlock)
k_count_live_tiles(const float* __restrict__ approx_poses, uint32_t kb, uint32_t nb, const float* __restrict__ tile_bounds, uint32_t n_tiles,
                   const uint32_t* __restrict__ smax_bits, float thr, unsigned long long* __restrict__ live)
{
    const uint32_t tile = blockIdx.x * blockDim.x + threadIdx.x;
    const uint32_t kfb = blockIdx.y;
    bool alive = false;
    if (tile < n_tiles) alive = !tile_out_of_reach(approx_poses + 16 * (size_t)(kb + kfb), tile_bounds + 6 * (size_t)tile, u2f(smax_bits[kfb]), thr);
    __shared__ uint32_t wsum[kBlock / 64];
    const uint64_t b = __builtin_amdgcn_ballot_w64(alive);
    if ((threadIdx.x & 63u) == 0u) wsum[threadIdx.x >> 6] = (uint32_t)__popcll(b);
    __syncthreads();
    if (threadIdx.x == 0) {
        uint32_t t = 0;
        for (int w = 0; w < kBlock / 64; ++w) t += wsum[w];
        if (t) atomicAdd(live, (unsigned long long)t);
    }
}
hipError_t count_live_tiles(const float* approx_poses_dev, size_t kb, size_t nb, const float* tile_bounds_dev, size_t n_tiles,
                            const uint32_t* smax_bits_dev, float thr, unsigned long long* live_dev, hipStream_t s)
{
    if (!nb || !n_tiles) return hipSuccess;
    k_count_live_tiles<<<dim3(grid_for(n_tiles), (unsigned)nb), dim3(kBlock), 0, s>>>(approx_poses_dev, (uint32_t)kb, (uint32_t)nb, tile_bounds_dev,
                                                                                    (uint32_t)n_tiles, smax_bits_dev, thr, live_dev);
    return hipGetLastError();
}

static constexpr int kCullSlots = 512;

template <bool B2L_IDENTITY, bool EL3>
__global__ void __launch_bounds__(kBlock) __attribute__((amdgpu_waves_per_eu(8, 8)))
k_vote_map_cull(const float4* __restrict__ map, uint32_t M, const double* __restrict__ inv_poses, const float* __restrict__ approx_poses,
                uint32_t kb, uint32_t nb, HostMat34 b2l_h, ProjLaunch pl, const float* __restrict__ qbound_img,
                const float* __restrict__ tile_bounds, const uint32_t* __restrict__ smax_bits, float thr, uint64_t* __restrict__ img)
{
    __shared__ uint64_t vals[kCullSlots];
    __shared__ uint32_t tags[kCullSlots];
    __shared__ uint32_t queue[kCullQueue];
    __shared__ uint16_t uqueue[kCullQueue];
    __shared__ uint32_t qcount, ucount;
    const uint32_t per_block = (uint32_t)(kBlock * kPtsPerThread);
    const TileKf tk = tile_kf_of_block(blockIdx.x, pl, nb);
    if (!tk.valid) return;
    if (tile_bounds && tile_out_of_reach(approx_poses + 16 * (size_t)(kb + tk.kfb), tile_bounds + 6 * (size_t)tk.tile, u2f(smax_bits[tk.kfb]), thr)) return;
    for (int s = threadIdx.x; s < kCullSlots; s += kBlock) { tags[s] = kEmptyTag; vals[s] = ~0ull; }
    if (threadIdx.x == 0) { qcount = 0; ucount = 0; }
    __syncthreads();
    const RimgGeom& g = pl.g;
    const uint32_t npx = pl.npx;
    const uint32_t block_base = tk.tile * per_block;
    const float4* __restrict__ mapb = map + block_base;
    const uint32_t nloc = min(per_block, M - block_base);
    const uint32_t kf = kb + tk.kfb;
    uint64_t* __restrict__ imgk = img + (size_t)tk.kfb * npx;
    const float* __restrict__ qk = qbound_img + (size_t)tk.kfb * npx;
    const float* __restrict__ ap = approx_poses + 16 * (size_t)kf;
    const bool full_tile = (nloc == per_block) & pl.packable & (ap[15] != 0.0f);
    if (full_tile) {
        constexpr int kInFlight = 4;
        constexpr bool kPrefetch = true;
        float4 nxt[kInFlight];
        if (kPrefetch) {
#pragma unroll
            for (int u = 0; u < kInFlight; ++u) nxt[u] = mapb[(uint32_t)u * kBlock + threadIdx.x];
        }
        const uint32_t lane_word = threadIdx.x << 20;
#pragma unroll
        for (uint32_t j0 = 0; j0 < (uint32_t)kPtsPerThread; j0 += kInFlight) {
            float4 pt[kInFlight];
            CullCand cc[kInFlight];
            float q0[kInFlight];
#pragma unroll
            for (int u = 0; u < kInFlight; ++u) {
                const uint32_t li = (j0 + u) * kBlock + threadIdx.x;
                if (kPrefetch) {
                    pt[u] = nxt[u];
                    if (j0 + kInFlight < (uint32_t)kPtsPerThread) nxt[u] = mapb[li + kInFlight * kBlock];
                } else {
                    pt[u] = mapb[li];
                }
            }
#pragma unroll
            for (int u = 0; u < kInFlight; ++u) {
                bool ok;
                const float3 p = xform_approx(ap, pt[u], ok);
                cc[u] = cull_candidates<EL3>(pl, p);
                cc[u].unusual |= cc[u].multi | (B2L_IDENTITY ? false : (cc[u].r2 < pl.rmin2));
                q0[u] = *reinterpret_cast<const float*>(reinterpret_cast<const char*>(qk) + ((__umul24((uint32_t)cc[u].rb, (uint32_t)g.cols) + (uint32_t)cc[u].cb) << 2));
            }
            bool mt[kInFlight];
#pragma unroll
            for (int u = 0; u < kInFlight; ++u) {
                mt[u] = cc[u].unusual | (cc[u].r2 < q0[u]);
            }
            const uint64_t b0 = __builtin_amdgcn_ballot_w64(mt[0]), b1 = __builtin_amdgcn_ballot_w64(mt[1]),
                           b2 = __builtin_amdgcn_ballot_w64(mt[2]), b3 = __builtin_amdgcn_ballot_w64(mt[3]);
            const uint32_t n0 = (uint32_t)__popcll(b0), n1 = (uint32_t)__popcll(b1), n2 = (uint32_t)__popcll(b2), n3 = (uint32_t)__popcll(b3);
            const uint32_t total = n0 + n1 + n2 + n3;
            if (total) {
                uint32_t base = 0;
                if ((threadIdx.x & 63u) == 0u) base = atomicAdd(&qcount, total);
                base = (uint32_t)__builtin_amdgcn_readfirstlane((int)base);
                if (base + total <= (uint32_t)kCullQueue) {
                    const uint64_t bal[kInFlight] = {b0, b1, b2, b3};
                    const uint32_t off[kInFlight] = {0u, n0, n0 + n1, n0 + n1 + n2};
#pragma unroll
                    for (int u = 0; u < kInFlight; ++u) {
                        if (!mt[u]) continue;
                        const uint32_t below = __builtin_amdgcn_mbcnt_hi((uint32_t)(bal[u] >> 32), __builtin_amdgcn_mbcnt_lo((uint32_t)bal[u], 0u));
                        const uint32_t rowq = cc[u].unusual ? 511u : (uint32_t)cc[u].rb;
                        queue[base + off[u] + below] = (((rowq << 11) | (uint32_t)cc[u].cb) | lane_word) | (((j0 + u) * kBlock) << 20);
                    }
                }
            }
        }
    }
    __syncthreads();
    const uint32_t nq_all = full_tile ? qcount : (uint32_t)kCullQueue + 1u;
    if (nloc == per_block && threadIdx.x == 0 && (blockIdx.x & 63u) == 0u) {
        atomicAdd(&g_cull_stats[0], (unsigned long long)nq_all);
        atomicAdd(&g_cull_stats[1], (unsigned long long)nloc);
    }
    if (nq_all) {
        const Mat34 Tinv = load_mat(inv_poses + 12 * (size_t)kf);
        if (__builtin_expect(nq_all > (uint32_t)kCullQueue, 0)) {
            for (uint32_t li = threadIdx.x; li < nloc; li += kBlock)
                exact_insert<B2L_IDENTITY, 8, 64>(map, block_base + li, Tinv, b2l_h, g, vals, tags, imgk);
        } else {
            for (uint32_t q = threadIdx.x; q < nq_all; q += kBlock) {
                const uint32_t e = queue[q];
                const int row = (int)((e >> 11) & 511u), col = (int)(e & 2047u);
                if (row == 511) { uqueue[atomicAdd(&ucount, 1u)] = (uint16_t)(e >> 20); continue; }
                const uint32_t i = block_base + (e >> 20);
                const uint32_t px = (uint32_t)(row * g.cols + col);
                const uint64_t v = ((uint64_t)exact_range_bits<B2L_IDENTITY>(map[i], Tinv, b2l_h) << 32) | (uint64_t)i;
                const int slot = table_claim<8, 64>(tags, row, col, px);
                if (slot >= 0) { if (v < vals[slot]) atomicMin(reinterpret_cast<unsigned long long*>(&vals[slot]), (unsigned long long)v); }
                else img_min_u64(imgk + px, v);
            }
            __syncthreads();
            const uint32_t nu = ucount;
            for (uint32_t q = threadIdx.x; q < nu; q += kBlock)
                exact_insert<B2L_IDENTITY, 8, 64>(map, block_base + uqueue[q], Tinv, b2l_h, g, vals, tags, imgk);
        }
    }
    __syncthreads();
    if (nq_all)
        for (int s = threadIdx.x; s < kCullSlots; s += kBlock) {
            const uint32_t t = tags[s];
            if (t != kEmptyTag) img_min_u64(imgk + t, vals[s]);
        }
}

hipError_t cull_stats(unsigned long long* out2, int reset, hipStream_t s, int which_kernel)
{
    hipError_t e = hipMemcpyFromSymbolAsync(out2, HIP_SYMBOL(g_cull_stats), 16, 16 * (size_t)(which_kernel ? 1 : 0), hipMemcpyDeviceToHost, s);
    if (e != hipSuccess) return e;
    e = hipStreamSynchronize(s);
    if (e != hipSuccess || !reset) return e;
    const unsigned long long z[4] = {0, 0, 0, 0};
    e = hipMemcpyToSymbolAsync(HIP_SYMBOL(g_cull_stats), z, 32, 0, hipMemcpyHostToDevice, s);
    return e == hipSuccess ? hipStreamSynchronize(s) : e;
}


hipError_t vote_map_range_images(const float4* map, size_t M, const double* inv_poses_dev, const float* approx_poses_dev, size_t kb, size_t nb,
                                 HostMat34 b2l, int b2l_identity, Geom g, const float* qbound_img, const float* tile_bounds_dev,
                                 const uint32_t* smax_bits_dev, float thr, int mode, uint64_t* map_img, hipStream_t s, const KernelOpts& ko)
{
    if (!M || !nb) return hipSuccess;
    if (mode != 0 || !ko.vote_cull || !approx_poses_dev || !qbound_img) return map_range_images(map, M, inv_poses_dev, approx_poses_dev, kb, nb, b2l, b2l_identity, g, map_img, s, ko);
    const size_t per_block = (size_t)kBlock * kPtsPerThread;
    dim3 grid(tile_kf_grid((M + per_block - 1) / per_block, nb));
    const ProjLaunch pl = make_proj_launch(g, b2l, b2l_identity, M);
    const float* tb = (ko.tile_cull && smax_bits_dev) ? tile_bounds_dev : nullptr;
    const bool el3 = g.el_fit != 0;
#define LTM_LAUNCH_CULL(ID, E) k_vote_map_cull<ID, E><<<grid, dim3(kBlock), 0, s>>>(map, (uint32_t)M, inv_poses_dev, approx_poses_dev, (uint32_t)kb, (uint32_t)nb, b2l, pl, qbound_img, tb, smax_bits_dev, thr, map_img)
    if (!b2l_identity) { if (el3) LTM_LAUNCH_CULL(false, true); else LTM_LAUNCH_CULL(false, false); }
    else { if (el3) LTM_LAUNCH_CULL(true, true); else LTM_LAUNCH_CULL(true, false); }
#undef LTM_LAUNCH_CULL
    return hipGetLastError();
}

__global__ void __launch_bounds__(kBlock)
k_cull_check(const float* __restrict__ xyz, size_t n, HostMat34 T, HostMat34 b2l, int b2l_identity, const float* __restrict__ ap, ProjLaunch pl,
             unsigned long long* __restrict__ bad)
{
    const size_t i = (size_t)blockIdx.x * blockDim.x + threadIdx.x;
    if (i >= n) return;
    const RimgGeom& g = pl.g;
    const float4 p4 = make_float4(xyz[3 * i], xyz[3 * i + 1], xyz[3 * i + 2], 0.0f);
    float3 pe = make_float3(p4.x, p4.y, p4.z), pa = pe;
    bool ok = true;
    if (ap) {
        pe = xform(to_dev(T), pe);
        pe = b2l_identity ? xform_identity(pe) : xform(to_dev(b2l), pe);
        pa = xform_approx(ap, p4, ok);
    }
    CullCand cc = g.el_fit ? cull_candidates<true>(pl, pa) : cull_candidates<false>(pl, pa);
    if (cc.unusual || !ok) return;
    if (ap && !b2l_identity && cc.r2 < pl.rmin2) return;
    if (cc.multi) cull_expand(pl, cc);
    const Sph s = cart2sph(pe.x, pe.y, pe.z);
    int row, col;
    pixel_row_col(g, s.az, s.el, row, col);
    const double re2 = (double)s.r * (double)s.r;
    const float r_lo = cull_r_lo(cc.r2);
    const bool good = (row == cc.r0 || row == cc.r1) && (col == cc.c0 || col == cc.c1) && (r_lo <= s.r) && (s.r <= r_lo * (1.0f + 3.0e-6f)) &&
                      (re2 >= (double)cc.r2 * (1.0 - 3.0e-6)) && (re2 <= (double)cc.r2 * (1.0 + 3.0e-6));
    if (!good) atomicAdd(bad, 1ull);
}
hipError_t cull_check(const float* xyz_dev, size_t n, const HostMat34* T, const HostMat34* b2l, int b2l_identity, const float* approx_pose_dev,
                      Geom g, unsigned long long* bad_dev, hipStream_t s)
{
    if (!n) return hipSuccess;
    HostMat34 z{};
    const int ident = b2l ? b2l_identity : 1;
    k_cull_check<<<dim3(grid_for(n)), dim3(kBlock), 0, s>>>(xyz_dev, n, T ? *T : z, b2l ? *b2l : z, ident,
                                                            T ? approx_pose_dev : nullptr, make_proj_launch(g, b2l ? *b2l : z, ident, 0), bad_dev);
    return hipGetLastError();
}

__global__ void __launch_bounds__(kBlock)
k_cull_probe_points(Geom g, size_t n, HostMat34 pose, int with_pose, float* __restrict__ xyz)
{
    const size_t i = (size_t)blockIdx.x * blockDim.x + threadIdx.x;
    if (i >= n) return;
    uint32_t h = (uint32_t)i * 0x9e3779b1u + 0x7f4a7c15u;
    auto next = [&]() { h ^= h >> 16; h *= 0x85ebca6bu; h ^= h >> 13; h *= 0xc2b2ae35u; h ^= h >> 16; return h; };
    const double jit[8] = {0.0, 1.0e-5, -1.0e-5, 1.0e-4, -1.0e-4, 4.0e-4, -4.0e-4, 2.0e-3};
    const double ranges[8] = {0.3, 1.0, 3.0, 10.0, 30.0, 60.0, 119.0, 200.0};
    const uint32_t kind = next() & 3u;
    double rowf = (double)(next() % (uint32_t)(g.rows * 16 + 1)) / 16.0 - 0.5;
    double colf = (double)(next() % (uint32_t)(g.cols * 16 + 1)) / 16.0 - 0.5;
    if (kind == 0 || kind == 2) rowf = (double)(next() % (uint32_t)(g.rows + 1)) - 0.5 + jit[next() & 7u];
    if (kind == 1 || kind == 2) colf = (double)(next() % (uint32_t)(g.cols + 1)) - 0.5 + jit[next() & 7u];
    const double el = ((double)g.vfov * 0.5 - (double)g.vfov * rowf / (double)g.rows) * (3.14159265358979323846 / 180.0);
    const double az = ((double)g.hfov * colf / (double)g.cols - (double)g.hfov * 0.5) * (3.14159265358979323846 / 180.0);
    const double r = ranges[next() & 7u] * (1.0 + 1.0e-3 * (double)(next() & 1023u));
    double x = r * cos(el) * cos(az), y = r * cos(el) * sin(az), z = r * sin(el);
    if (with_pose) {
        const double X = pose.m[0] * x + pose.m[1] * y + pose.m[2] * z + pose.m[3], Y = pose.m[4] * x + pose.m[5] * y + pose.m[6] * z + pose.m[7],
                     Z = pose.m[8] * x + pose.m[9] * y + pose.m[10] * z + pose.m[11];
        x = X; y = Y; z = Z;
    }
    xyz[3 * i] = (float)x; xyz[3 * i + 1] = (float)y; xyz[3 * i + 2] = (float)z;
}
hipError_t cull_probe_points(Geom g, size_t n, const HostMat34* pose, float* xyz_dev, hipStream_t s)
{
    if (!n) return hipSuccess;
    HostMat34 z{};
    k_cull_probe_points<<<dim3(grid_for(n)), dim3(kBlock), 0, s>>>(g, n, pose ? *pose : z, pose ? 1 : 0, xyz_dev);
    return hipGetLastError();
}

static constexpr int kBmSlotsMax = 1024;
static constexpr int kBmQueue = 2048;
static constexpr uint32_t kBmRowUncertain = 511u;
static constexpr int kBmUQueue = 1024;


template <bool B2L_IDENTITY, bool EL3, int SLOT_ROWS = 16>
__global__ void __launch_bounds__(kBlock)
k_map_rimg_blockmin(const float4* __restrict__ map, uint32_t M, const double* __restrict__ inv_poses, const float* __restrict__ approx_poses,
                    uint32_t kb, uint32_t nb, HostMat34 b2l_h, ProjLaunch pl, uint64_t* __restrict__ img, const uint32_t* __restrict__ pairs, uint32_t n_pairs,
                    const uint8_t* __restrict__ submask)
{
    constexpr int kBmSlots = SLOT_ROWS * 64;
    static_assert(kBmSlots <= kBmSlotsMax, "");
    __shared__ uint64_t vals[kBmSlots];
    __shared__ uint32_t tags[kBmSlots];
    uint32_t* const amin = reinterpret_cast<uint32_t*>(vals);
    __shared__ uint32_t queue[kBmQueue];
    __shared__ uint16_t uqueue[kBmUQueue];
    __shared__ uint32_t qcount, ucount;
    const uint32_t per_block = (uint32_t)(kBlock * kPtsPerThread);
    TileKf tk;
    uint32_t quarters = 0xfu;
    if (pairs) {
        const uint32_t seg = (n_pairs + 7u) >> 3, at = (blockIdx.x & 7u) * seg + (blockIdx.x >> 3);
        if ((blockIdx.x >> 3) >= seg || at >= n_pairs) return;
        const uint32_t pr = pairs[at];
        tk.tile = (uint32_t)__builtin_amdgcn_readfirstlane((int)(pr / nb)); tk.kfb = (uint32_t)__builtin_amdgcn_readfirstlane((int)(pr % nb)); tk.valid = true;
        if (submask) quarters = (uint32_t)__builtin_amdgcn_readfirstlane((int)submask[pr]);
    } else {
        tk = tile_kf_of_block(blockIdx.x, pl, nb);
    }
    if (!tk.valid) return;
    for (int s = threadIdx.x; s < kBmSlots; s += kBlock) { tags[s] = kEmptyTag; amin[s] = 0x7f800000u; }
    if (threadIdx.x == 0) { qcount = 0; ucount = 0; }
    __syncthreads();
    const RimgGeom& g = pl.g;
    const uint32_t npx = pl.npx;
    const uint32_t block_base = tk.tile * per_block;
    const float4* __restrict__ mapb = map + block_base;
    const uint32_t nloc = min(per_block, M - block_base);
    const uint32_t kf = kb + tk.kfb;
    uint64_t* __restrict__ imgk = img + (size_t)tk.kfb * npx;
    const float* __restrict__ ap = approx_poses + 16 * (size_t)kf;
    static_assert(kBmRowUncertain == 511u, "ProjLaunch::packable is rows < 511");
    float rlo[kPtsPerThread];
    uint32_t rec[kPtsPerThread];
    const bool full_tile = (nloc == per_block) & pl.packable & (ap[15] != 0.0f);
    if (full_tile) {
#pragma unroll
        for (int j0 = 0; j0 < kPtsPerThread; j0 += 4) {
            if (!((quarters >> (j0 >> 2)) & 1u)) {
#pragma unroll
                for (int u = 0; u < 4; ++u) { rlo[j0 + u] = -1.0f; rec[j0 + u] = 0u; }
                continue;
            }
            float4 pt[4];
            CullCand cc[4];
#pragma unroll
            for (int u = 0; u < 4; ++u) pt[u] = mapb[(uint32_t)(j0 + u) * kBlock + threadIdx.x];
#pragma unroll
            for (int u = 0; u < 4; ++u) {
                bool ok;
                const float3 p = xform_approx(ap, pt[u], ok);
                cc[u] = cull_candidates<EL3>(pl, p);
            }
#pragma unroll
            for (int u = 0; u < 4; ++u) {
                const int j = j0 + u;
                const float r_lo = cull_r_lo(cc[u].r2);
                rlo[j] = -1.0f;
                const bool certain = !cc[u].unusual & !cc[u].multi & !(cc[u].r2 < pl.rmin2);
                rec[j] = ((certain ? (uint32_t)cc[u].rb : kBmRowUncertain) << 11) | (uint32_t)(cc[u].cb & 2047);
                if (!certain) continue;
                const uint32_t px = (uint32_t)(cc[u].rb * g.cols + cc[u].cb);
// ... 260 lines not shown
    dim3 grid((unsigned)(((n_pairs + 7) / 8) * 8));
    const ProjLaunch pl = make_proj_launch(g, b2l, b2l_identity, M);
#define LTM_LAUNCH_BMP(ID, E) k_map_rimg_blockmin<ID, E><<<grid, dim3(kBlock), 0, s>>>(map, (uint32_t)M, inv_poses_dev, approx_poses_dev, (uint32_t)kb, (uint32_t)nb, b2l, pl, map_img, pairs, (uint32_t)n_pairs, submask)
    const bool el3 = g.el_fit != 0;
    if (!b2l_identity) { if (el3) LTM_LAUNCH_BMP(false, true); else LTM_LAUNCH_BMP(false, false); }
    else { if (el3) LTM_LAUNCH_BMP(true, true); else LTM_LAUNCH_BMP(true, false); }
#undef LTM_LAUNCH_BMP
    return hipGetLastError();
}

__global__ void __launch_bounds__(kBlock)
k_compare_flag(const uint32_t* __restrict__ scan_img, const uint64_t* __restrict__ map_img, size_t n, float thr, int mode,
               uint8_t* __restrict__ labels)
{
    const size_t i = (size_t)blockIdx.x * blockDim.x + threadIdx.x;
    if (i >= n) return;
    const uint64_t mv = map_img[i];
    const float map_r = u2f((uint32_t)(mv >> 32));
    const float scan_r = u2f(scan_img[i]);
    const float diff = (mode == 0) ? (scan_r - map_r) : (map_r - scan_r);
    if (diff < 200.0f  && diff > thr) labels[(uint32_t)mv] = 1;
}

hipError_t compare_and_flag(const uint32_t* scan_img, const uint64_t* map_img, size_t n, float thr, int mode, uint8_t* labels,
                            hipStream_t s)
{
    if (!n) return hipSuccess;
    k_compare_flag<<<dim3(grid_for(n)), dim3(kBlock), 0, s>>>(scan_img, map_img, n, thr, mode, labels);
    return hipGetLastError();
}

__global__ void __launch_bounds__(kBlock)
k_single_rimg(const float4* __restrict__ pts, size_t n, HostMat34 T1, int has1, HostMat34 T2, int has2, Geom gg,
              uint64_t* __restrict__ img)
{
    const size_t i = (size_t)blockIdx.x * blockDim.x + threadIdx.x;
    if (i >= n) return;
    const RimgGeom g = make_geom(gg);
    const float4 p4 = pts[i];
    float3 p = make_float3(p4.x, p4.y, p4.z);
    if (has1) p = xform(to_dev(T1), p);
    if (has2) p = xform(to_dev(T2), p);
    const Sph s = cart2sph(p.x, p.y, p.z);
    const int px = pixel_index(g, s.az, s.el);
    img_min_u64(img + px, ((uint64_t)f2u(s.r) << 32) | (uint64_t)(uint32_t)i);
}

hipError_t single_range_image(const float4* pts, size_t n, const HostMat34* T1, const HostMat34* T2, Geom g, uint64_t* img,
                              hipStream_t s)
{
    if (!n) return hipSuccess;
    HostMat34 z{};
    k_single_rimg<<<dim3(grid_for(n)), dim3(kBlock), 0, s>>>(pts, n, T1 ? *T1 : z, T1 != nullptr, T2 ? *T2 : z, T2 != nullptr, g, img);
    return hipGetLastError();
}

__global__ void k_decode_image(const uint64_t* img, size_t npx, float* rimg, int32_t* ptidx)
{
    const size_t i = (size_t)blockIdx.x * blockDim.x + threadIdx.x;
    if (i >= npx) return;
    const uint64_t v = img[i];
    rimg[i] = u2f((uint32_t)(v >> 32));
    if (ptidx) ptidx[i] = (int32_t)(uint32_t)v;
}
hipError_t decode_image(const uint64_t* img, size_t npx, float* rimg, int32_t* ptidx, hipStream_t s)
{
    k_decode_image<<<dim3(grid_for(npx)), dim3(kBlock), 0, s>>>(img, npx, rimg, ptidx);
    return hipGetLastError();
}

__global__ void k_debug_project(const float* xyz, size_t n, Geom gg, float* sph, int32_t* rc)
{
    const size_t i = (size_t)blockIdx.x * blockDim.x + threadIdx.x;
    if (i >= n) return;
    const RimgGeom g = make_geom(gg);
    const Sph s = cart2sph(xyz[3 * i], xyz[3 * i + 1], xyz[3 * i + 2]);
    sph[3 * i] = s.az; sph[3 * i + 1] = s.el; sph[3 * i + 2] = s.r;
    const int px = pixel_index(g, s.az, s.el);
    rc[2 * i] = px / g.cols; rc[2 * i + 1] = px % g.cols;
}
hipError_t debug_project(const float* xyz_dev, size_t n, Geom g, float* az_el_r, int32_t* row_col, hipStream_t s)
{
    if (!n) return hipSuccess;
    k_debug_project<<<dim3(grid_for(n)), dim3(kBlock), 0, s>>>(xyz_dev, n, g, az_el_r, row_col);
    return hipGetLastError();
}

__global__ void __launch_bounds__(kBlock)
k_selfcheck(float vfov, float hfov, unsigned long long* __restrict__ counts)
{
    const float inv_v = 1.0f / vfov, inv_h = 1.0f / hfov;
    unsigned long long bad0 = 0, bad1 = 0, bad2 = 0;
    const uint64_t stride = (uint64_t)gridDim.x * blockDim.x;
    for (uint64_t i = (uint64_t)blockIdx.x * blockDim.x + threadIdx.x; i < (1ull << 32); i += stride) {
        const float a = u2f((uint32_t)i);
        const float e0 = rad2deg_exact(a), f0 = rad2deg_fast(a);
        const float e1 = a / vfov, f1 = div_by_const(a, vfov, inv_v, true);
        const float e2 = a / hfov, f2 = div_by_const(a, hfov, inv_h, true);
        bad0 += !((f2u(e0) == f2u(f0)) | ((e0 != e0) & (f0 != f0)));
        bad1 += !((f2u(e1) == f2u(f1)) | ((e1 != e1) & (f1 != f1)));
        bad2 += !((f2u(e2) == f2u(f2)) | ((e2 != e2) & (f2 != f2)));
    }
    if (bad0) atomicAdd(counts + 0, bad0);
    if (bad1) atomicAdd(counts + 1, bad1);
    if (bad2) atomicAdd(counts + 2, bad2);
}
hipError_t selfcheck_fast_math(float vfov, float hfov, unsigned long long* counts_dev, hipStream_t s)
{
    k_selfcheck<<<dim3(8192), dim3(kBlock), 0, s>>>(vfov, hfov, counts_dev);
    return hipGetLastError();
}

static void proj_launch_flatten(const ProjLaunch& pl, uint32_t nb, float* f, uint32_t* u)
{
    const RimgGeom& g = pl.g;
    const float ff[kProjLaunchFloats] = {g.half_v, g.half_h, g.inv_v, g.inv_h, g.frows, g.fcols, g.row_max, g.col_max, pl.row_scale, pl.col_scale,
                                         pl.row_bias, pl.col_bias, pl.certain_lim, pl.rmin2, g.eps, g.el_tclamp};
    const uint32_t uu[kProjLaunchWords] = {(uint32_t)g.rows, (uint32_t)g.cols, pl.npx, pl.steep_clamps ? 1u : 0u, pl.packable ? 1u : 0u, pl.n_tiles, pl.n_tg,
                                           pl.tg_magic, pl.tg_shift, tile_kf_grid(pl.n_tiles, nb), g.el_fit ? 1u : 0u, g.fast ? 1u : 0u};
    memcpy(f, ff, sizeof ff);
    memcpy(u, uu, sizeof uu);
}
__global__ void k_proj_launch_eval(Geom gg, HostMat34 b2l, int b2l_identity, size_t M, ProjLaunch* out)
{
    if (blockIdx.x == 0 && threadIdx.x == 0) *out = make_proj_launch(gg, b2l, b2l_identity, M);
}
hipError_t proj_launch_debug(Geom g, HostMat34 b2l, int b2l_identity, size_t M, size_t nb, int on_device, float* f, uint32_t* u)
{
    ProjLaunch pl = make_proj_launch(g, b2l, b2l_identity, M);
    if (on_device) {
        ProjLaunch* d = nullptr;
        hipError_t e = hipMalloc(reinterpret_cast<void**>(&d), sizeof(ProjLaunch));
        if (e != hipSuccess) return e;
        k_proj_launch_eval<<<dim3(1), dim3(64)>>>(g, b2l, b2l_identity, M, d);
        e = hipGetLastError();
        if (e == hipSuccess) e = hipMemcpy(&pl, d, sizeof(ProjLaunch), hipMemcpyDeviceToHost);
        (void)hipFree(d);
        if (e != hipSuccess) return e;
    }
    proj_launch_flatten(pl, (uint32_t)nb, f, u);
    return hipSuccess;
}
void proj_launch_blocks(size_t M, size_t nb, uint32_t first_block, size_t n, uint32_t* tile, uint32_t* kf)
{
    Geom g{};
    g.vfov = g.hfov = 1.0f;
    const ProjLaunch pl = make_proj_launch(g, HostMat34{}, 1, M);
    for (size_t i = 0; i < n; ++i) {
        const TileKf t = tile_kf_of_block(first_block + (uint32_t)i, pl, (uint32_t)nb);
        tile[i] = t.valid ? t.tile : 0xffffffffu;
        kf[i] = t.valid ? t.kfb : 0xffffffffu;
    }
}

}
```

### lt-mapper_amd/csrc/ltm_kernels.h

```cpp
#pragma once
#include <hip/hip_runtime_api.h>
#include <stddef.h>
#include <stdint.h>

namespace ltm {

struct Geom {
    float vfov, hfov;
    int rows, cols;
    int fast;
    float cull_eps_px;
    int el_fit;
    float el_c[4];
    float el_tclamp;
};

struct HostMat34 { double m[12]; };

static const uint32_t kNoPointBits = 0x461C4000u;

hipError_t fill_u32(uint32_t* p, uint32_t v, size_t n, hipStream_t s);
hipError_t fill_u64(uint64_t* p, uint64_t v, size_t n, hipStream_t s);

hipError_t scan_range_images(const float4* scans, const uint64_t* offsets_dev, size_t kb, size_t nb,
                             uint64_t first_pt, uint64_t n_pts, uint64_t max_kf_pts, Geom g, uint32_t* scan_img, uint32_t* smax_bits, hipStream_t s);
static constexpr int kMaxScanShapes = 8;
hipError_t scan_range_images_multi(const float4* scans, const uint64_t* offsets_dev, size_t kb, size_t nb, uint64_t n_pts, uint64_t max_kf_pts, Geom g,
                                   int n_shapes, const int* rows, const int* cols, uint32_t* const* imgs, uint32_t* const* smax_bits, hipStream_t s);
hipError_t scan_qbound(const uint32_t* scan_img, size_t n, float thr, float* qbound, hipStream_t s);
hipError_t tile_bounds(const float4* map, size_t M, float* bounds, hipStream_t s);
hipError_t subtile_bounds(const float4* map, size_t M, float* bounds, hipStream_t s);
struct KernelOpts {
    int map_kernel_variant = 2;
    int vote_cull = 1;
    int tile_cull = 1;
    int stats_blockmin = 0;
};
hipError_t map_range_images(const float4* map, size_t M, const double* inv_poses_dev, const float* approx_poses_dev, size_t kb, size_t nb,
                            HostMat34 b2l, int b2l_identity, Geom g, uint64_t* map_img, hipStream_t s, const KernelOpts& ko);
hipError_t occlusion_shell_pairs(const float* approx_poses_dev, size_t kb, size_t nb, const float* tile_bounds_dev, size_t n_tiles, Geom g, float r_lo, float r_hi,
                                 const uint64_t* img, int use_cmax, uint32_t* cmax, uint8_t* done, uint8_t* flags, uint32_t* pos, uint32_t* list, uint32_t* count,
                                 void* temp, size_t temp_bytes, hipStream_t s, uint32_t* dirty_rows = nullptr,
                                 const float* sub_bounds_dev = nullptr, uint8_t* submask = nullptr, unsigned long long* sub_stats = nullptr);
hipError_t map_range_images_pairs(const float4* map, size_t M, const double* inv_poses_dev, const float* approx_poses_dev, size_t kb, size_t nb,
                                  HostMat34 b2l, int b2l_identity, Geom g, uint64_t* map_img, const uint32_t* pairs, size_t n_pairs, hipStream_t s, const KernelOpts& ko,
                                  const uint8_t* submask = nullptr);
hipError_t compare_and_flag(const uint32_t* scan_img, const uint64_t* map_img, size_t n_px_total, float thr, int mode,
                            uint8_t* labels, hipStream_t s);
hipError_t vote_map_range_images(const float4* map, size_t M, const double* inv_poses_dev, const float* approx_poses_dev, size_t kb, size_t nb,
                                 HostMat34 b2l, int b2l_identity, Geom g, const float* qbound_img, const float* tile_bounds_dev,
                                 const uint32_t* smax_bits_dev, float thr, int mode, uint64_t* map_img, hipStream_t s, const KernelOpts& ko);
hipError_t count_live_tiles(const float* approx_poses_dev, size_t kb, size_t nb, const float* tile_bounds_dev, size_t n_tiles,
                            const uint32_t* smax_bits_dev, float thr, unsigned long long* live_dev, hipStream_t s);
static constexpr int kProjLaunchFloats = 16, kProjLaunchWords = 12;
hipError_t proj_launch_debug(Geom g, HostMat34 b2l, int b2l_identity, size_t M, size_t nb, int on_device, float* f, uint32_t* u);
void proj_launch_blocks(size_t M, size_t nb, uint32_t first_block, size_t n, uint32_t* tile, uint32_t* kf);
hipError_t cull_stats(unsigned long long* out2, int reset, hipStream_t s, int which_kernel);
hipError_t cull_check(const float* xyz_dev, size_t n, const HostMat34* T, const HostMat34* b2l, int b2l_identity, const float* approx_pose_dev,
                      Geom g, unsigned long long* bad_dev, hipStream_t s);
hipError_t cull_probe_points(Geom g, size_t n, const HostMat34* pose, float* xyz_dev, hipStream_t s);
hipError_t single_range_image(const float4* pts, size_t n, const HostMat34* T1, const HostMat34* T2, Geom g,
                              uint64_t* img, hipStream_t s);
hipError_t decode_image(const uint64_t* img, size_t npx, float* rimg, int32_t* ptidx, hipStream_t s);
hipError_t viz_diff(const uint32_t* scan_bits, const float* map_r, size_t n, int mode, float* out, hipStream_t s);
hipError_t viz_colormap_f32(const float* src, size_t n, float a, float b, const uint8_t* lut, uint8_t* bgr, hipStream_t s);
hipError_t viz_colormap_i32(const int32_t* src, size_t n, double a, double b, const uint8_t* lut, uint8_t* bgr, hipStream_t s);
hipError_t debug_project(const float* xyz_dev, size_t n, Geom g, float* az_el_r, int32_t* row_col, hipStream_t s);
hipError_t selfcheck_fast_math(float vfov, float hfov, unsigned long long* counts_dev, hipStream_t s);

size_t scan_temp_bytes(size_t n);
hipError_t exclusive_scan_u8(const uint8_t* labels, uint32_t* pos, size_t n, void* temp, size_t temp_bytes, hipStream_t s);
hipError_t exclusive_scan_img_valid(const uint64_t* img, uint32_t* pos, size_t n, void* temp, size_t temp_bytes, hipStream_t s);
hipError_t exclusive_scan_u32(const uint32_t* in, uint32_t* out, size_t n, void* temp, size_t temp_bytes, hipStream_t s);
hipError_t partition_scatter(const float4* in, const uint8_t* labels, const uint32_t* pos, size_t n,
                             float4* kept, float4* flagged, hipStream_t s);
hipError_t reproject_gather(const uint64_t* img, const uint32_t* pos, size_t npx, size_t nb, const float4* map,
                            const double* inv_poses_dev, size_t kb, HostMat34 b2l, int b2l_identity,
                            float4* out, hipStream_t s);
hipError_t image_bounds(const uint32_t* pos, const uint64_t* img, size_t npx, size_t nb, uint32_t* out, hipStream_t s);
hipError_t flag_bounds(const uint32_t* pos, const uint8_t* flag, size_t n, const uint64_t* offsets_dev, size_t kf0, uint64_t first, size_t nb,
                       uint32_t* out, hipStream_t s);
hipError_t gather_u32(const uint32_t* in, const uint64_t* idx_dev, size_t m, size_t n, uint32_t tail_value_index_n,
                      uint32_t* out, hipStream_t s);

hipError_t transform_cloud(const float4* in, size_t n, const HostMat34* t1, const HostMat34* t2, float4* out, hipStream_t s);
hipError_t transform_scans(const float4* in, const uint64_t* offsets_dev, size_t n_kf, uint64_t n_pts,
                           HostMat34 first, int first_identity, const double* per_kf_dev, float4* out, hipStream_t s);
hipError_t zip_concat(const float4* a, const uint64_t* oa, const float4* b, const uint64_t* ob, const float4* c, const uint64_t* oc,
                      const uint64_t* out_off_dev, size_t n_kf, uint64_t n, float4* out, hipStream_t s);
hipError_t preclean_flags(const float4* in, uint64_t n, float radius, uint8_t* keep, hipStream_t s);

hipError_t bbox_init(uint32_t* bbox, hipStream_t s);
hipError_t bbox_reduce(const float4* pts, size_t n, uint32_t* bbox, hipStream_t s);
struct OctreeFrame { double minx, miny, minz, res; unsigned depth; };
hipError_t bbox_reduce_check(const float4* pts, size_t n, OctreeFrame cached_frame, uint32_t* bbox8, hipStream_t s);
size_t voxel_heads_starts_temp_bytes(size_t n);
hipError_t voxel_heads_starts(const uint64_t* sorted_keys, size_t n, unsigned shift, uint32_t* starts, void* temp, uint32_t* total_out_dev, hipStream_t s);
hipError_t morton_keys(const float4* pts, size_t n, OctreeFrame f, uint64_t* keys, uint32_t* idx, hipStream_t s);
hipError_t bbox_reduce_seg(const float4* pts, const uint64_t* offsets_dev, size_t n_kf, uint64_t n, uint32_t* bbox, hipStream_t s);
hipError_t morton_keys_seg(const float4* pts, const uint64_t* offsets_dev, size_t n_kf, uint64_t n, const OctreeFrame* frames_dev,
                           unsigned shift, uint64_t* keys, uint32_t* idx, hipStream_t s);
struct VoxelGridFrame { float inv; int min_b[3]; int div_b[3]; int passthrough; };
hipError_t voxelgrid_keys_seg(const float4* pts, const uint64_t* offsets_dev, size_t n_kf, uint64_t n, const VoxelGridFrame* frames_dev,
                              uint64_t* keys, uint32_t* idx, hipStream_t s);
hipError_t voxelgrid_centroids(const float4* pts, const uint64_t* sorted_keys, const uint32_t* sorted_idx, const uint32_t* starts,
                               const VoxelGridFrame* frames_dev, size_t n_vox, size_t n, float4* out, hipStream_t s);
size_t sort_temp_bytes(size_t n);
hipError_t scan_total_to(const uint8_t* flags, const uint32_t* pos, size_t n, uint32_t* out_dev, hipStream_t s);
hipError_t sort_pairs_u64(const uint64_t* keys_in, uint64_t* keys_out, const uint32_t* val_in, uint32_t* val_out, size_t n,
                          unsigned end_bit, void* temp, size_t temp_bytes, hipStream_t s);
hipError_t head_flags(const uint64_t* keys, size_t n, uint8_t* heads, hipStream_t s, unsigned shift = 0);
static constexpr int kMaxKeyRuns = 24;
struct KeyCompress { int n_runs; unsigned bits; unsigned char src[kMaxKeyRuns], dst[kMaxKeyRuns]; uint64_t mask[kMaxKeyRuns]; };
hipError_t morton_keys_packed(const float4* pts, size_t n, OctreeFrame f, KeyCompress kc, unsigned idx_bits, uint64_t* keys, hipStream_t s);
size_t sort_keys_temp_bytes(size_t n);
hipError_t sort_keys_u64(const uint64_t* keys_in, uint64_t* keys_out, size_t n, unsigned begin_bit, unsigned end_bit, void* temp,
                         size_t temp_bytes, hipStream_t s);
hipError_t voxel_centroids_packed(const float4* pts, const uint64_t* sorted_keys, uint64_t idx_mask, const uint32_t* starts, size_t n_vox,
                                  size_t n, float4* out, hipStream_t s);
hipError_t compact_keys(const uint64_t* keys, const uint8_t* flags, const uint32_t* pos, size_t n, uint64_t* keys_out, hipStream_t s);
static constexpr int kVoxelKeyBins = 4096;
hipError_t key_histogram(const uint64_t* keys, size_t n, unsigned shift, uint32_t* hist, hipStream_t s);
hipError_t key_range_flags(const uint64_t* keys, size_t n, uint64_t lo, uint64_t hi, uint8_t* flags, hipStream_t s);
hipError_t compact_pairs(const uint64_t* keys, const uint32_t* idx, const uint8_t* flags, const uint32_t* pos, size_t n,
                         uint64_t* keys_out, uint32_t* idx_out, hipStream_t s);
hipError_t segment_starts(const uint8_t* heads, const uint32_t* pos, size_t n, uint32_t* starts, hipStream_t s);
hipError_t voxel_centroids(const float4* pts, const uint32_t* sorted_idx, const uint32_t* starts, size_t n_vox, size_t n,
                           float4* out, hipStream_t s);

struct KnnGrid { double ox, oy, oz, inv_cell; long long nx, ny, nz; };
hipError_t cell_keys(const float4* pts, size_t n, KnnGrid g, uint64_t* keys, uint32_t* idx, hipStream_t s);
hipError_t gather_points(const float4* in, const uint32_t* idx, size_t n, float4* out, hipStream_t s);
hipError_t gather_u64(const uint64_t* in, const uint32_t* idx, size_t n, uint64_t* out, hipStream_t s);
struct HashEntry { uint64_t key; uint32_t start, end; };
hipError_t hash_build(const uint64_t* sorted_keys, const uint32_t* starts, size_t n_cells, size_t n_pts,
                      HashEntry* table, uint32_t table_mask, hipStream_t s);
hipError_t knn_query_scans(const float4* scans, const uint64_t* offsets_dev, size_t kb, size_t ke, uint64_t first_pt, uint64_t n_pts, uint64_t max_kf_pts,
                           const double* poses_dev, const double* inv_poses_dev, HostMat34 b2l, int b2l_identity,
                           const float4* sorted_target, size_t Mt, KnnGrid g, const HashEntry* table, uint32_t table_mask,
                           int k, float thr, float cell2_lo, uint8_t* coexist, float4* local_out, hipStream_t s);
hipError_t knn_bucket_build(const float4* sorted_target, const uint64_t* sorted_keys, const uint32_t* starts, size_t n_cells, size_t n_pts, KnnGrid g,
                            void* buckets, uint32_t n_buckets, hipStream_t s);
hipError_t knn_bitmap_build(const uint64_t* sorted_keys, const uint32_t* starts, size_t n_cells, KnnGrid g, void* occ_words, uint32_t word_mask, hipStream_t s);
hipError_t knn_two_phase_fast(const float4* scans, const uint64_t* offsets_dev, size_t kb, size_t ke, uint64_t first_pt, uint64_t n_pts, uint64_t max_kf_pts,
                              const double* poses_dev, const double* inv_poses_dev, HostMat34 b2l, int b2l_identity, KnnGrid g, const void* buckets,
                              uint32_t n_buckets, int k, float thr, uint8_t* coexist, float4* local_out, hipStream_t s,
                              float4* gp_undecided = nullptr);
hipError_t knn_two_phase_exact(const float4* scans, const uint64_t* offsets_dev, size_t kb, size_t ke, uint64_t first_pt, uint64_t n_pts,
                               const double* poses_dev, HostMat34 b2l, int b2l_identity, const float4* sorted_target, size_t Mt, KnnGrid g,
                               const HashEntry* table, uint32_t table_mask, const void* bitmap, uint32_t bitmap_mask, int k, float thr, float cell2_lo, uint8_t* coexist,
                               uint32_t* pos, uint32_t* queue, uint32_t* count, void* temp, size_t temp_bytes, hipStream_t s);
unsigned knn_sorted_queue_bits(KnnGrid g, uint64_t n_pts, unsigned* ibits_out);
hipError_t knn_two_phase_compact_keyed(const float4* scans, const uint64_t* offsets_dev, size_t kb, size_t ke, uint64_t first_pt, uint64_t n_pts, const double* poses_dev,
                                       HostMat34 b2l, int b2l_identity, KnnGrid g, unsigned ibits, const uint8_t* flags, uint32_t* pos, uint64_t* queue, uint32_t* count,
                                       void* temp, size_t temp_bytes, hipStream_t s, const float4* gp_undecided = nullptr);
hipError_t knn_two_phase_exact_sorted(const float4* scans, const uint64_t* offsets_dev, size_t kb, size_t ke, uint64_t first_pt, const double* poses_dev, HostMat34 b2l,
                                      int b2l_identity, const float4* sorted_target, size_t Mt, KnnGrid g, const HashEntry* table, uint32_t table_mask, const void* bitmap,
                                      uint32_t bitmap_mask, int k, float thr, float cell2_lo, uint8_t* coexist, const uint64_t* queue_in, uint64_t* queue_sorted, uint32_t n_und,
                                      unsigned ibits, unsigned kbits, void* temp, size_t temp_bytes, hipStream_t s, const float4* gp_undecided = nullptr);
hipError_t knn_query_cloud(const float4* query, size_t Q, const float4* sorted_target, size_t Mt, KnnGrid g,
                           const HashEntry* table, uint32_t table_mask, int k, float thr, float cell2_lo,
                           uint8_t* near, hipStream_t s);

static constexpr int kSearchLeaf = 32;
struct SearchFrame { double ox, oy, oz, scale; };
struct SearchTree { const float4* pts; const uint32_t* idx; const uint64_t* keys; const float4* box; uint32_t Mf, L, P; };
hipError_t search_bbox(const float4* pts, size_t n, uint32_t* bbox8, hipStream_t s);
hipError_t search_keys(const float4* pts, size_t n, SearchFrame f, uint64_t* keys, uint32_t* idx, hipStream_t s);
hipError_t search_tree_boxes(const float4* sorted_pts, uint32_t Mf, uint32_t L, uint32_t P, float4* box, hipStream_t s);
hipError_t search_query_order(const float4* query, size_t n, SearchFrame f, uint64_t* keys, uint64_t* keys_sorted, uint32_t* idx, uint32_t* order,
                              void* temp, size_t temp_bytes, hipStream_t s);
hipError_t knn_search(const float4* query, size_t n, const uint32_t* order, const uint64_t* qkeys_sorted, SearchTree t, int k,
                      int32_t* out_idx, float* out_d2, hipStream_t s);
hipError_t knn_empty_rows(size_t n, int32_t* idx, float* d2, hipStream_t s);
hipError_t radius_count(const float4* query, size_t n, const uint32_t* order, SearchTree t, float r2, uint32_t* count, hipStream_t s);
size_t     radius_scan_temp_bytes(size_t n);
hipError_t radius_offsets(const uint32_t* count, size_t n, uint32_t cap, uint64_t* off, void* temp, size_t temp_bytes, hipStream_t s);
size_t     radius_sort_temp_bytes(size_t total, size_t n);
hipError_t radius_fill(const float4* query, size_t n, const uint32_t* order, SearchTree t, float r2, const uint64_t* full_off, uint64_t total_full,
                       const uint64_t* out_off, uint64_t* pairs, uint64_t* pairs_sorted, int32_t* out_idx, float* out_d2, void* temp, size_t temp_bytes, hipStream_t s);

static constexpr int kSearchSegChunk = 1024;
struct SearchSeg { SearchFrame f; const float4* src; uint64_t first, box0; uint32_t n, Mf, L, P, block0, pad; };
hipError_t search_bbox_seg(const SearchSeg* segs, size_t n_segs, const uint32_t* block_seg, uint32_t n_blocks, uint32_t* bbox8, hipStream_t s);
hipError_t search_keys_seg(const SearchSeg* segs, const uint32_t* block_seg, uint32_t n_blocks, uint64_t* keys, uint32_t* idx, hipStream_t s);
size_t     search_sort_seg_temp_bytes(size_t total, size_t n_segs);
hipError_t search_sort_gather_seg(const SearchSeg* segs, const uint32_t* block_seg, uint32_t n_blocks, size_t n_segs, const uint64_t* offsets, size_t total,
                                  const uint64_t* keys, uint64_t* keys_sorted, const uint32_t* idx, uint32_t* order, float4* sorted, void* temp,
                                  size_t temp_bytes, hipStream_t s);
hipError_t search_tree_boxes_seg(const SearchSeg* segs, size_t n_segs, const float4* sorted, float4* box, hipStream_t s);

static constexpr int kNormalsBlockReg = 256;
static constexpr int kNormalsBlockLds = 64;
static constexpr int kNormalsMaxK = 64;
struct NormalsSeg { SearchTree t; float4* out; double vp[3]; uint32_t block0, pad; };
int        normals_block(int k);
hipError_t estimate_normals(const NormalsSeg* segs, const uint32_t* block_seg, uint32_t n_blocks, int k, hipStream_t s);

struct SubmapPiece { uint64_t src, dst; uint32_t n, block0, affine, pad; };
hipError_t submap_gather(const float4* scans, const SubmapPiece* pieces, const uint32_t* block_piece, uint32_t n_blocks, const float* affines12, float4* out,
                         hipStream_t s);

static constexpr int kIcpBlock = 256;
static constexpr int kIcpPartial = 17;
static constexpr int kIcpPlanePartial = 29;
enum IcpMode { kIcpPoint = 0, kIcpScore = 1, kIcpPlane = 2 };
struct IcpPair { SearchTree t; SearchFrame f; const float4* src; double o[3]; uint64_t first; uint32_t n, block0, n_blocks, pad; const float4* nrm; };
struct IcpState { double T[12]; double prev_mse, last_mse, fitness; int32_t iterations, state, converged, done; uint32_t n_corr, pad; };
hipError_t icp_source_keys(const IcpPair* pairs, const uint32_t* block_pair, uint32_t n_blocks, uint64_t* keys, uint32_t* idx, hipStream_t s);
// ... 23 lines not shown
```

### lt-mapper_amd/csrc/ltm_kernels_common.h

```cpp
#pragma once
#include "ltm_kernels.h"
#include "ltm_device_math.h"
#include "ltm_device_prims.h"

#include <algorithm>
#include <cstring>
#include <type_traits>
#include <hip/hip_runtime.h>

namespace ltm {

static constexpr int kBlock = 256;

__host__ __device__ inline RimgGeom make_geom(Geom g)
{
    RimgGeom r;
    r.vfov = g.vfov; r.hfov = g.hfov;
    r.half_v = g.vfov / 2.0f; r.half_h = g.hfov / 2.0f;
    r.inv_v = 1.0f / g.vfov; r.inv_h = 1.0f / g.hfov;
    r.fast = g.fast != 0;
    r.eps = g.cull_eps_px;
    r.el_c0 = g.el_c[0]; r.el_c1 = g.el_c[1]; r.el_c2 = g.el_c[2]; r.el_c3 = g.el_c[3]; r.el_tclamp = g.el_tclamp; r.el_fit = g.el_fit != 0;
    r.rows = g.rows; r.cols = g.cols;
    r.frows = (float)g.rows; r.fcols = (float)g.cols;
    r.row_max = (float)(g.rows - 1); r.col_max = (float)(g.cols - 1);
    return r;
}

static constexpr unsigned kKfPerTile = 8;
struct ProjLaunch {
    RimgGeom g;
    float row_scale, col_scale;
    float row_bias, col_bias;
    float certain_lim;
    float rmin2;
    uint32_t npx;
    uint32_t n_tiles, n_tg;
    uint32_t tg_magic, tg_shift;
    bool steep_clamps;
    bool packable;
};
__host__ __device__ inline ProjLaunch make_proj_launch(Geom gg, const HostMat34& b2l, int b2l_identity, size_t M)
{
    ProjLaunch pl;
    const RimgGeom g = make_geom(gg);
    pl.g = g;
    pl.row_scale = g.frows * (57.29577951308232f / g.vfov); pl.col_scale = g.fcols * (57.29577951308232f / g.hfov);
    pl.row_bias = 0.5f * g.frows + 0.5f - g.eps; pl.col_bias = 0.5f * g.fcols + 0.5f - g.eps;
    pl.certain_lim = 1.0f - 2.0f * g.eps;
    float rmin = 0.0f;
    if (!b2l_identity) {
        const float tx = (float)b2l.m[3], ty = (float)b2l.m[7], tz = (float)b2l.m[11];
        rmin = 0.125f * __builtin_sqrtf(tx * tx + ty * ty + tz * tz) + 1.0e-6f;
    }
    pl.rmin2 = rmin * rmin;
    pl.npx = (uint32_t)(g.rows * g.cols);
    pl.steep_clamps = g.vfov < 88.0f;
    pl.packable = g.rows < 511 && g.cols <= 2048;
    const size_t per_block = (size_t)kBlock * 16;
    pl.n_tiles = (uint32_t)((M + per_block - 1) / per_block);
    pl.n_tg = (pl.n_tiles + 7u) >> 3;
    const uint32_t d = pl.n_tg ? pl.n_tg : 1u;
    uint32_t s = 0;
    while (((uint64_t)1 << s) < d) ++s;
    pl.tg_shift = s;
    pl.tg_magic = (uint32_t)((((uint64_t)1 << (26u + s)) / d) + 1u);
    return pl;
}

struct TileKf { uint32_t tile, kfb; bool valid; };
__host__ __device__ inline TileKf tile_kf_of_block(uint32_t b, const ProjLaunch& pl, uint32_t nb)
{
    static_assert(kKfPerTile == 8, "the shifts below are log2(8 XCDs) + log2(kKfPerTile)");
    const uint32_t x = b & 7u, kfl = (b >> 3) & (kKfPerTile - 1u), q = b >> 6;
    const uint32_t kg = (uint32_t)(((uint64_t)(b & ~63u) * pl.tg_magic) >> 32) >> pl.tg_shift;
    const uint32_t tg = q - kg * pl.n_tg;
    TileKf t;
    t.tile = tg * 8u + x;
    t.kfb = kg * kKfPerTile + kfl;
    t.valid = (t.tile < pl.n_tiles) & (t.kfb < nb);
    return t;
}
static inline unsigned tile_kf_grid(size_t n_tiles, size_t nb)
{
    const size_t n_tg = (n_tiles + 7) / 8, n_kg = (nb + kKfPerTile - 1) / kKfPerTile;
    return (unsigned)(n_tg * 8 * kKfPerTile * n_kg);
}

inline unsigned grid_for(size_t n, int block = kBlock)
{
    size_t b = (n + block - 1) / block;
    return (unsigned)(b == 0 ? 1 : b);
}

__device__ __forceinline__ Mat34 load_mat(const double* p)
{
    Mat34 T;
#pragma unroll
    for (int i = 0; i < 12; ++i) T.m[i] = p[i];
    return T;
}
__device__ __forceinline__ Mat34 to_dev(const HostMat34& h)
{
    Mat34 T;
#pragma unroll
    for (int i = 0; i < 12; ++i) T.m[i] = h.m[i];
    return T;
}

__device__ __forceinline__ void img_min_u64(uint64_t* p, uint64_t v)
{
    const uint64_t cur = __hip_atomic_load(p, __ATOMIC_RELAXED, __HIP_MEMORY_SCOPE_AGENT);
    if (v < cur) atomicMin(reinterpret_cast<unsigned long long*>(p), (unsigned long long)v);
}
__device__ __forceinline__ void img_min_u32(uint32_t* p, uint32_t v)
{
    const uint32_t cur = __hip_atomic_load(p, __ATOMIC_RELAXED, __HIP_MEMORY_SCOPE_AGENT);
    if (v < cur) atomicMin(p, v);
}

__device__ __forceinline__ size_t find_kf(const uint64_t* __restrict__ offsets, size_t lo, size_t hi, uint64_t gi)
{
    while (hi - lo > 1) {
        const size_t mid = (lo + hi) >> 1;
        if (offsets[mid] <= gi) lo = mid; else hi = mid;
    }
    return lo;
}

}
```

Baseline: 3249 keyframe-pairs/s.

## Process runs of consecutive map tiles per block in vote cull kernel

The vote-map cull kernel now assigns each block a run of up to T consecutive tiles (default 4) for one keyframe instead of a single tile. Tiles are pre-filtered with one ballot, and the shared-memory hash table and unusual-point queue are kept across tiles, so the table flush to global memory happens once per run. This is meant to cut per-block setup cost, the number of redundant global atomicMin flushes, and launch grid size. In exchange there are fewer blocks, which may hurt occupancy and load balance, and uqueue entries now pack a tile offset into 16 bits.

```diff
diff --git a/include/ltm.h b/include/ltm.h
--- a/include/ltm.h
+++ b/include/ltm.h
@@ -212,6 +212,8 @@
 int ltm_debug_voxel_key_bits(const float* mn3, const float* mx3, float leaf, uint64_t* kept_mask, unsigned* depth, double* frame_min3);
 int ltm_debug_proj_launch(float vfov, float hfov, float res_alpha, const double* base2lidar16_or_null, size_t map_points, size_t n_keyframes, int on_device,
                           float* out_f32, uint32_t* out_u32, uint32_t first_block, size_t n_blocks, uint32_t* out_tile, uint32_t* out_kf);
+int ltm_debug_vote_run_launch(size_t map_points, size_t n_keyframes, int tile_run, uint32_t first_block, size_t n_blocks, uint32_t* out_run, uint32_t* out_kf,
+                              uint32_t* out_run_len, uint32_t* out_grid);
 int ltm_debug_cull_check(ltm_ctx*, const float* xyz, size_t n, const double* inv_pose16_or_null, float res_alpha, uint64_t* violations);
 int ltm_debug_cull_validation(ltm_ctx*, uint64_t* shapes_checked, uint64_t* shapes_failed);
 int ltm_debug_occlusion_stats(ltm_ctx*, uint64_t* pairs, uint64_t* first_shell, uint64_t* projected, int reset);
diff --git a/lt-mapper_amd/capi.py b/lt-mapper_amd/capi.py
--- a/lt-mapper_amd/capi.py
+++ b/lt-mapper_amd/capi.py
@@ -158,6 +158,7 @@
     "ltm_debug_cull_check": (_i, [_vp, _vp, _sz, _vp, _f, _pu64]),
     "ltm_debug_cull_stats": (_i, [_vp, _pu64, _pu64, _i]),
     "ltm_debug_proj_launch": (_i, [_f, _f, _f, _vp, _sz, _sz, _i, _vp, _vp, C.c_uint32, _sz, _vp, _vp]),
+    "ltm_debug_vote_run_launch": (_i, [_sz, _sz, _i, C.c_uint32, _sz, _vp, _vp, _vp, _vp]),
     "ltm_debug_cull_validation": (_i, [_vp, _pu64, _pu64]),
     "ltm_debug_occlusion_stats": (_i, [_vp, _pu64, _pu64, _pu64, _i]),
     "ltm_debug_voxel_stats": (_i, [_vp, _pu64, _pu64, _i]),
@@ -220,6 +221,17 @@
     if rc != 0:
         raise LtmError(rc, "ltm_debug_proj_launch")
     return dict(zip(PROJ_LAUNCH_F32, f)), {k: int(v) for k, v in zip(PROJ_LAUNCH_U32, u)}, tile[:n_blocks], kf[:n_blocks]
+
+
+def vote_run_launch(map_points, n_keyframes, tile_run, first_block=0, n_blocks=0):
+    run = np.zeros(max(n_blocks, 1), dtype=np.uint32)
+    kf = np.zeros(max(n_blocks, 1), dtype=np.uint32)
+    run_len, grid = C.c_uint32(0), C.c_uint32(0)
+    rc = load_library().ltm_debug_vote_run_launch(int(map_points), int(n_keyframes), int(tile_run), int(first_block), int(n_blocks), run.ctypes.data,
+                                                  kf.ctypes.data, C.byref(run_len), C.byref(grid))
+    if rc != 0:
+        raise LtmError(rc, "ltm_debug_vote_run_launch")
+    return run[:n_blocks], kf[:n_blocks], run_len.value, grid.value
 
 
 def inverse4x4(m):
diff --git a/lt-mapper_amd/csrc/ltm_api_core.cpp b/lt-mapper_amd/csrc/ltm_api_core.cpp
--- a/lt-mapper_amd/csrc/ltm_api_core.cpp
+++ b/lt-mapper_amd/csrc/ltm_api_core.cpp
@@ -217,6 +217,7 @@
     c->kopts.map_kernel_variant = env_int("LTM_MAP_KERNEL", 2);
     c->kopts.vote_cull = env_int("LTM_VOTE_CULL", 1);
     c->kopts.tile_cull = env_int("LTM_TILE_CULL", 1);
+    c->kopts.vote_tile_run = std::min(std::max(env_int("LTM_VOTE_TILE_RUN", 4), 1), 16);
     c->kopts.stats_blockmin = env_int("LTM_STATS_BLOCKMIN", 0);
     {
         unsigned long long* d = nullptr;
diff --git a/lt-mapper_amd/csrc/ltm_api_vote.cpp b/lt-mapper_amd/csrc/ltm_api_vote.cpp
--- a/lt-mapper_amd/csrc/ltm_api_vote.cpp
+++ b/lt-mapper_amd/csrc/ltm_api_vote.cpp
@@ -287,7 +287,7 @@
             }
             ProfScope p(c, cull ? "vote_map_cull" : "vote_map_exact", pts, bytes, bytes_c);
             if (cull) {
-                HeavyScope hs(c, n_tiles * nb);
+                HeavyScope hs(c, vote_run_blocks(map.n, nb, c->kopts.vote_tile_run));
                 LTM_HIP(vote_map_range_images(map.d, map.n, ps.inv_dev, ps.approx_dev, kb, nb, c->B2L, c->b2l_identity, g, qbound, tb.as<float>(), smax, thr, mode,
                                               map_img.as<uint64_t>(), hs.stream(), c->kopts));
                 hs.done();
@@ -573,6 +573,17 @@
     return LTM_OK;
 }
 
+int ltm_debug_vote_run_launch(size_t map_points, size_t n_keyframes, int tile_run, uint32_t first_block, size_t n_blocks, uint32_t* out_run, uint32_t* out_kf,
+                              uint32_t* out_run_len, uint32_t* out_grid)
+{
+    if (map_points >= 0xffffffffull || n_keyframes >= 0xffffffffull || tile_run < 1 || (n_blocks && (!out_run || !out_kf))) return LTM_E_INVALID;
+    uint32_t len = 0;
+    const unsigned grid = vote_run_launch_blocks(map_points, n_keyframes, tile_run, first_block, n_blocks, out_run, out_kf, &len);
+    if (out_run_len) *out_run_len = len;
+    if (out_grid) *out_grid = grid;
+    return LTM_OK;
+}
+
 int ltm_debug_cull_stats(ltm_ctx* c, uint64_t* survivors, uint64_t* points, int reset)
 {
     return guarded(c, [&] {
diff --git a/lt-mapper_amd/csrc/ltm_k_projection.hip b/lt-mapper_amd/csrc/ltm_k_projection.hip
--- a/lt-mapper_amd/csrc/ltm_k_projection.hip
+++ b/lt-mapper_amd/csrc/ltm_k_projection.hip
@@ -443,7 +443,7 @@
 template <bool B2L_IDENTITY, bool EL3>
 __global__ void __launch_bounds__(kBlock) __attribute__((amdgpu_waves_per_eu(8, 8)))
 k_vote_map_cull(const float4* __restrict__ map, uint32_t M, const double* __restrict__ inv_poses, const float* __restrict__ approx_poses,
-                uint32_t kb, uint32_t nb, HostMat34 b2l_h, ProjLaunch pl, const float* __restrict__ qbound_img,
+                uint32_t kb, uint32_t nb, HostMat34 b2l_h, ProjLaunch pl, RunLaunch rl, const float* __restrict__ qbound_img,
                 const float* __restrict__ tile_bounds, const uint32_t* __restrict__ smax_bits, float thr, uint64_t* __restrict__ img)
 {
     __shared__ uint64_t vals[kCullSlots];
@@ -451,117 +451,152 @@
     __shared__ uint32_t queue[kCullQueue];
     __shared__ uint16_t uqueue[kCullQueue];
     __shared__ uint32_t qcount, ucount;
+    static_assert(kMaxTileRun * kBlock * kPtsPerThread <= 65536, "uqueue entries are 16 bits");
     const uint32_t per_block = (uint32_t)(kBlock * kPtsPerThread);
-    const TileKf tk = tile_kf_of_block(blockIdx.x, pl, nb);
-    if (!tk.valid) return;
-    if (tile_bounds && tile_out_of_reach(approx_poses + 16 * (size_t)(kb + tk.kfb), tile_bounds + 6 * (size_t)tk.tile, u2f(smax_bits[tk.kfb]), thr)) return;
+    const RunKf rk = run_kf_of_block(blockIdx.x, rl, nb);
+    if (!rk.valid) return;
+    const RimgGeom& g = pl.g;
+    const uint32_t npx = pl.npx;
+    const uint32_t kf = kb + rk.kfb;
+    const uint32_t first_tile = rk.run * rl.T;
+    const uint32_t run_base = first_tile * per_block;
+    uint64_t* __restrict__ imgk = img + (size_t)rk.kfb * npx;
+    const float* __restrict__ qk = qbound_img + (size_t)rk.kfb * npx;
+    const float* __restrict__ ap = approx_poses + 16 * (size_t)kf;
+    uint32_t todo;
+    {
+        const uint32_t t = threadIdx.x & 63u;
+        bool visit = (t < rl.T) & (first_tile + t < pl.n_tiles);
+        if (visit && tile_bounds) visit = !tile_out_of_reach(ap, tile_bounds + 6 * (size_t)(first_tile + t), u2f(smax_bits[rk.kfb]), thr);
+        todo = (uint32_t)__builtin_amdgcn_ballot_w64(visit);
+    }
+    if (!todo) return;
     for (int s = threadIdx.x; s < kCullSlots; s += kBlock) { tags[s] = kEmptyTag; vals[s] = ~0ull; }
     if (threadIdx.x == 0) { qcount = 0; ucount = 0; }
     __syncthreads();
-    const RimgGeom& g = pl.g;
-    const uint32_t npx = pl.npx;
-    const uint32_t block_base = tk.tile * per_block;
-    const float4* __restrict__ mapb = map + block_base;
-    const uint32_t nloc = min(per_block, M - block_base);
-    const uint32_t kf = kb + tk.kfb;
-    uint64_t* __restrict__ imgk = img + (size_t)tk.kfb * npx;
-    const float* __restrict__ qk = qbound_img + (size_t)tk.kfb * npx;
-    const float* __restrict__ ap = approx_poses + 16 * (size_t)kf;
-    const bool full_tile = (nloc == per_block) & pl.packable & (ap[15] != 0.0f);
-    if (full_tile) {
-        constexpr int kInFlight = 4;
-        constexpr bool kPrefetch = true;
-        float4 nxt[kInFlight];
-        if (kPrefetch) {
-#pragma unroll
-            for (int u = 0; u < kInFlight; ++u) nxt[u] = mapb[(uint32_t)u * kBlock + threadIdx.x];
-        }
-        const uint32_t lane_word = threadIdx.x << 20;
-#pragma unroll
-        for (uint32_t j0 = 0; j0 < (uint32_t)kPtsPerThread; j0 += kInFlight) {
-            float4 pt[kInFlight];
-            CullCand cc[kInFlight];
-            float q0[kInFlight];
-#pragma unroll
-            for (int u = 0; u < kInFlight; ++u) {
-                const uint32_t li = (j0 + u) * kBlock + threadIdx.x;
-                if (kPrefetch) {
-                    pt[u] = nxt[u];
-                    if (j0 + kInFlight < (uint32_t)kPtsPerThread) nxt[u] = mapb[li + kInFlight * kBlock];
-                } else {
-                    pt[u] = mapb[li];
+    const bool fast_ok = pl.packable & ((f2u(ap[15]) << 1) != 0u);
+    const double* __restrict__ inv_pose = inv_poses + 12 * (size_t)kf;
+    bool flush = false;
+    uint32_t qbase = 0;
+    for (; todo; todo &= todo - 1u) {
+        const uint32_t tile = first_tile + (uint32_t)__builtin_ctz(todo);
+        const uint32_t block_base = tile * per_block;
+        const float4* __restrict__ mapb = map + block_base;
+        const uint32_t nloc = min(per_block, M - block_base);
+        const bool full_tile = (nloc == per_block) & fast_ok;
+        if (full_tile) {
+            constexpr int kInFlight = 4;
+            constexpr bool kPrefetch = true;
+            float4 nxt[kInFlight];
+            if (kPrefetch) {
+#pragma unroll
+                for (int u = 0; u < kInFlight; ++u) nxt[u] = mapb[(uint32_t)u * kBlock + threadIdx.x];
+            }
+            const uint32_t lane_word = threadIdx.x << 20;
+#pragma unroll
+            for (uint32_t j0 = 0; j0 < (uint32_t)kPtsPerThread; j0 += kInFlight) {
+                float4 pt[kInFlight];
+                CullCand cc[kInFlight];
+                float q0[kInFlight];
+#pragma unroll
+                for (int u = 0; u < kInFlight; ++u) {
+                    const uint32_t li = (j0 + u) * kBlock + threadIdx.x;
+                    if (kPrefetch) {
+                        pt[u] = nxt[u];
+                        if (j0 + kInFlight < (uint32_t)kPtsPerThread) nxt[u] = mapb[li + kInFlight * kBlock];
+                    } else {
+                        pt[u] = mapb[li];
+                    }
                 }
-            }
-#pragma unroll
-            for (int u = 0; u < kInFlight; ++u) {
-                bool ok;
-                const float3 p = xform_approx(ap, pt[u], ok);
-                cc[u] = cull_candidates<EL3>(pl, p);
-                cc[u].unusual |= cc[u].multi | (B2L_IDENTITY ? false : (cc[u].r2 < pl.rmin2));
-                q0[u] = *reinterpret_cast<const float*>(reinterpret_cast<const char*>(qk) + ((__umul24((uint32_t)cc[u].rb, (uint32_t)g.cols) + (uint32_t)cc[u].cb) << 2));
-            }
-            bool mt[kInFlight];
-#pragma unroll
-            for (int u = 0; u < kInFlight; ++u) {
-                mt[u] = cc[u].unusual | (cc[u].r2 < q0[u]);
-            }
-            const uint64_t b0 = __builtin_amdgcn_ballot_w64(mt[0]), b1 = __builtin_amdgcn_ballot_w64(mt[1]),
-                           b2 = __builtin_amdgcn_ballot_w64(mt[2]), b3 = __builtin_amdgcn_ballot_w64(mt[3]);
-            const uint32_t n0 = (uint32_t)__popcll(b0), n1 = (uint32_t)__popcll(b1), n2 = (uint32_t)__popcll(b2), n3 = (uint32_t)__popcll(b3);
-            const uint32_t total = n0 + n1 + n2 + n3;
-            if (total) {
-                uint32_t base = 0;
-                if ((threadIdx.x & 63u) == 0u) base = atomicAdd(&qcount, total);
-                base = (uint32_t)__builtin_amdgcn_readfirstlane((int)base);
-                if (base + total <= (uint32_t)kCullQueue) {
-                    const uint64_t bal[kInFlight] = {b0, b1, b2, b3};
-                    const uint32_t off[kInFlight] = {0u, n0, n0 + n1, n0 + n1 + n2};
-#pragma unroll
-                    for (int u = 0; u < kInFlight; ++u) {
-                        if (!mt[u]) continue;
-                        const uint32_t below = __builtin_amdgcn_mbcnt_hi((uint32_t)(bal[u] >> 32), __builtin_amdgcn_mbcnt_lo((uint32_t)bal[u], 0u));
-                        const uint32_t rowq = cc[u].unusual ? 511u : (uint32_t)cc[u].rb;
-                        queue[base + off[u] + below] = (((rowq << 11) | (uint32_t)cc[u].cb) | lane_word) | (((j0 + u) * kBlock) << 20);
+#pragma unroll
+                for (int u = 0; u < kInFlight; ++u) {
+                    bool ok;
+                    const float3 p = xform_approx(ap, pt[u], ok);
+                    cc[u] = cull_candidates<EL3>(pl, p);
+                    cc[u].unusual |= cc[u].multi | (B2L_IDENTITY ? false : (cc[u].r2 < pl.rmin2));
+                    q0[u] = *reinterpret_cast<const float*>(reinterpret_cast<const char*>(qk) + ((__umul24((uint32_t)cc[u].rb, (uint32_t)g.cols) + (uint32_t)cc[u].cb) << 2));
+                }
+                bool mt[kInFlight];
+#pragma unroll
+                for (int u = 0; u < kInFlight; ++u) {
+                    mt[u] = cc[u].unusual | (cc[u].r2 < q0[u]);
+                }
+                const uint64_t b0 = __builtin_amdgcn_ballot_w64(mt[0]), b1 = __builtin_amdgcn_ballot_w64(mt[1]),
+                               b2 = __builtin_amdgcn_ballot_w64(mt[2]), b3 = __builtin_amdgcn_ballot_w64(mt[3]);
+                const uint32_t n0 = (uint32_t)__popcll(b0), n1 = (uint32_t)__popcll(b1), n2 = (uint32_t)__popcll(b2), n3 = (uint32_t)__popcll(b3);
+                const uint32_t total = n0 + n1 + n2 + n3;
+                if (total) {
+                    uint32_t base = 0;
+                    if ((threadIdx.x & 63u) == 0u) base = atomicAdd(&qcount, total);
+                    base = (uint32_t)__builtin_amdgcn_readfirstlane((int)base) - qbase;
+                    if (base + total <= (uint32_t)kCullQueue) {
+                        const uint64_t bal[kInFlight] = {b0, b1, b2, b3};
+                        const uint32_t off[kInFlight] = {0u, n0, n0 + n1, n0 + n1 + n2};
+#pragma unroll
+                        for (int u = 0; u < kInFlight; ++u) {
+                            if (!mt[u]) continue;
+                            const uint32_t below = __builtin_amdgcn_mbcnt_hi((uint32_t)(bal[u] >> 32), __builtin_amdgcn_mbcnt_lo((uint32_t)bal[u], 0u));
+                            const uint32_t rowq = cc[u].unusual ? 511u : (uint32_t)cc[u].rb;
+                            queue[base + off[u] + below] = (((rowq << 11) | (uint32_t)cc[u].cb) | lane_word) | (((j0 + u) * kBlock) << 20);
+                        }
                     }
                 }
             }
         }
+        const uint32_t nu_waiting = (uint32_t)__builtin_amdgcn_readfirstlane((int)ucount);
+        __syncthreads();
+        const uint32_t qend = (uint32_t)__builtin_amdgcn_readfirstlane((int)qcount);
+        const uint32_t nq_all = full_tile ? qend - qbase : (uint32_t)kCullQueue + 1u;
+        qbase = qend;
+        if (nloc == per_block && threadIdx.x == 0 && (blockIdx.x & 63u) == 0u) {
+            atomicAdd(&g_cull_stats[0], (unsigned long long)nq_all);
+            atomicAdd(&g_cull_stats[1], (unsigned long long)nloc);
+        }
+        if (nq_all) {
+            flush = true;
+            const Mat34 Tinv = load_mat(inv_pose);
+            if (__builtin_expect(nq_all > (uint32_t)kCullQueue, 0)) {
+                for (uint32_t li = threadIdx.x; li < nloc; li += kBlock)
+                    exact_insert<B2L_IDENTITY, 8, 64>(map, block_base + li, Tinv, b2l_h, g, vals, tags, imgk);
+            } else {
+                if (__builtin_expect(nu_waiting + nq_all > (uint32_t)kCullQueue, 0)) {
+                    uint32_t q0 = threadIdx.x;
+                    asm volatile("" : "+v"(q0));
+                    for (uint32_t q = q0; q < nu_waiting; q += kBlock)
+                        exact_insert<B2L_IDENTITY, 8, 64>(map, run_base + uqueue[q], Tinv, b2l_h, g, vals, tags, imgk);
+                    __syncthreads();
+                    if (threadIdx.x == 0) ucount = 0;
+                    __syncthreads();
+                }
+                const uint32_t tile_word = (tile - first_tile) << 12;
+                for (uint32_t q = threadIdx.x; q < nq_all; q += kBlock) {
+                    const uint32_t e = queue[q];
+                    const int row = (int)((e >> 11) & 511u), col = (int)(e & 2047u);
+                    if (row == 511) { uqueue[atomicAdd(&ucount, 1u)] = (uint16_t)(tile_word | (e >> 20)); continue; }
+                    const uint32_t i = block_base + (e >> 20);
+                    const uint32_t px = (uint32_t)(row * g.cols + col);
+                    const uint64_t v = ((uint64_t)exact_range_bits<B2L_IDENTITY>(map[i], Tinv, b2l_h) << 32) | (uint64_t)i;
+                    const int slot = table_claim<8, 64>(tags, row, col, px);
+                    if (slot >= 0) { if (v < vals[slot]) atomicMin(reinterpret_cast<unsigned long long*>(&vals[slot]), (unsigned long long)v); }
+                    else img_min_u64(imgk + px, v);
+                }
+            }
+        }
+        __builtin_amdgcn_s_waitcnt(0x0f70);
+        __syncthreads();
+    }
+    if (!flush) return;
+    const uint32_t nu = ucount;
+    if (nu) {
+        const Mat34 Tinv = load_mat(inv_pose);
+        for (uint32_t q = threadIdx.x; q < nu; q += kBlock)
+            exact_insert<B2L_IDENTITY, 8, 64>(map, run_base + uqueue[q], Tinv, b2l_h, g, vals, tags, imgk);
     }
     __syncthreads();
-    const uint32_t nq_all = full_tile ? qcount : (uint32_t)kCullQueue + 1u;
-    if (nloc == per_block && threadIdx.x == 0 && (blockIdx.x & 63u) == 0u) {
-        atomicAdd(&g_cull_stats[0], (unsigned long long)nq_all);
-        atomicAdd(&g_cull_stats[1], (unsigned long long)nloc);
-    }
-    if (nq_all) {
-        const Mat34 Tinv = load_mat(inv_poses + 12 * (size_t)kf);
-        if (__builtin_expect(nq_all > (uint32_t)kCullQueue, 0)) {
-            for (uint32_t li = threadIdx.x; li < nloc; li += kBlock)
-                exact_insert<B2L_IDENTITY, 8, 64>(map, block_base + li, Tinv, b2l_h, g, vals, tags, imgk);
-        } else {
-            for (uint32_t q = threadIdx.x; q < nq_all; q += kBlock) {
-                const uint32_t e = queue[q];
-                const int row = (int)((e >> 11) & 511u), col = (int)(e & 2047u);
-                if (row == 511) { uqueue[atomicAdd(&ucount, 1u)] = (uint16_t)(e >> 20); continue; }
-                const uint32_t i = block_base + (e >> 20);
-                const uint32_t px = (uint32_t)(row * g.cols + col);
-                const uint64_t v = ((uint64_t)exact_range_bits<B2L_IDENTITY>(map[i], Tinv, b2l_h) << 32) | (uint64_t)i;
-                const int slot = table_claim<8, 64>(tags, row, col, px);
-                if (slot >= 0) { if (v < vals[slot]) atomicMin(reinterpret_cast<unsigned long long*>(&vals[slot]), (unsigned long long)v); }
-                else img_min_u64(imgk + px, v);
-            }
-            __syncthreads();
-            const uint32_t nu = ucount;
-            for (uint32_t q = threadIdx.x; q < nu; q += kBlock)
-                exact_insert<B2L_IDENTITY, 8, 64>(map, block_base + uqueue[q], Tinv, b2l_h, g, vals, tags, imgk);
-        }
-    }
-    __syncthreads();
-    if (nq_all)
-        for (int s = threadIdx.x; s < kCullSlots; s += kBlock) {
-            const uint32_t t = tags[s];
-            if (t != kEmptyTag) img_min_u64(imgk + t, vals[s]);
-        }
+    for (int s = threadIdx.x; s < kCullSlots; s += kBlock) {
+        const uint32_t t = tags[s];
+        if (t != kEmptyTag) img_min_u64(imgk + t, vals[s]);
+    }
 }
 
 hipError_t cull_stats(unsigned long long* out2, int reset, hipStream_t s, int which_kernel)
@@ -582,12 +617,12 @@
 {
     if (!M || !nb) return hipSuccess;
     if (mode != 0 || !ko.vote_cull || !approx_poses_dev || !qbound_img) return map_range_images(map, M, inv_poses_dev, approx_poses_dev, kb, nb, b2l, b2l_identity, g, map_img, s, ko);
-    const size_t per_block = (size_t)kBlock * kPtsPerThread;
-    dim3 grid(tile_kf_grid((M + per_block - 1) / per_block, nb));
     const ProjLaunch pl = make_proj_launch(g, b2l, b2l_identity, M);
+    const RunLaunch rl = make_run_launch(pl.n_tiles, (uint32_t)std::max(ko.vote_tile_run, 1));
+    dim3 grid(run_kf_grid(rl, nb));
     const float* tb = (ko.tile_cull && smax_bits_dev) ? tile_bounds_dev : nullptr;
     const bool el3 = g.el_fit != 0;
-#define LTM_LAUNCH_CULL(ID, E) k_vote_map_cull<ID, E><<<grid, dim3(kBlock), 0, s>>>(map, (uint32_t)M, inv_poses_dev, approx_poses_dev, (uint32_t)kb, (uint32_t)nb, b2l, pl, qbound_img, tb, smax_bits_dev, thr, map_img)
+#define LTM_LAUNCH_CULL(ID, E) k_vote_map_cull<ID, E><<<grid, dim3(kBlock), 0, s>>>(map, (uint32_t)M, inv_poses_dev, approx_poses_dev, (uint32_t)kb, (uint32_t)nb, b2l, pl, rl, qbound_img, tb, smax_bits_dev, thr, map_img)
     if (!b2l_identity) { if (el3) LTM_LAUNCH_CULL(false, true); else LTM_LAUNCH_CULL(false, false); }
     else { if (el3) LTM_LAUNCH_CULL(true, true); else LTM_LAUNCH_CULL(true, false); }
 #undef LTM_LAUNCH_CULL
@@ -1154,5 +1189,22 @@
         kf[i] = t.valid ? t.kfb : 0xffffffffu;
     }
 }
-
-}
+size_t vote_run_blocks(size_t M, size_t nb, int tile_run)
+{
+    const size_t per_block = (size_t)kBlock * kPtsPerThread;
+    return (size_t)make_run_launch((uint32_t)((M + per_block - 1) / per_block), (uint32_t)std::max(tile_run, 1)).n_runs * nb;
+}
+unsigned vote_run_launch_blocks(size_t M, size_t nb, int tile_run, uint32_t first_block, size_t n, uint32_t* run, uint32_t* kf, uint32_t* run_len)
+{
+    const size_t per_block = (size_t)kBlock * kPtsPerThread;
+    const RunLaunch rl = make_run_launch((uint32_t)((M + per_block - 1) / per_block), (uint32_t)std::max(tile_run, 1));
+    for (size_t i = 0; i < n; ++i) {
+        const RunKf t = run_kf_of_block(first_block + (uint32_t)i, rl, (uint32_t)nb);
+        run[i] = t.valid ? t.run : 0xffffffffu;
+        kf[i] = t.valid ? t.kfb : 0xffffffffu;
+    }
+    if (run_len) *run_len = rl.T;
+    return run_kf_grid(rl, nb);
+}
+
+}
diff --git a/lt-mapper_amd/csrc/ltm_kernels.h b/lt-mapper_amd/csrc/ltm_kernels.h
--- a/lt-mapper_amd/csrc/ltm_kernels.h
+++ b/lt-mapper_amd/csrc/ltm_kernels.h
@@ -34,6 +34,7 @@
     int map_kernel_variant = 2;
     int vote_cull = 1;
     int tile_cull = 1;
+    int vote_tile_run = 4;
     int stats_blockmin = 0;
 };
 hipError_t map_range_images(const float4* map, size_t M, const double* inv_poses_dev, const float* approx_poses_dev, size_t kb, size_t nb,
@@ -55,6 +56,8 @@
 static constexpr int kProjLaunchFloats = 16, kProjLaunchWords = 12;
 hipError_t proj_launch_debug(Geom g, HostMat34 b2l, int b2l_identity, size_t M, size_t nb, int on_device, float* f, uint32_t* u);
 void proj_launch_blocks(size_t M, size_t nb, uint32_t first_block, size_t n, uint32_t* tile, uint32_t* kf);
+size_t vote_run_blocks(size_t M, size_t nb, int tile_run);
+unsigned vote_run_launch_blocks(size_t M, size_t nb, int tile_run, uint32_t first_block, size_t n, uint32_t* run, uint32_t* kf, uint32_t* run_len);
 hipError_t cull_stats(unsigned long long* out2, int reset, hipStream_t s, int which_kernel);
 hipError_t cull_check(const float* xyz_dev, size_t n, const HostMat34* T, const HostMat34* b2l, int b2l_identity, const float* approx_pose_dev,
                       Geom g, unsigned long long* bad_dev, hipStream_t s);
diff --git a/lt-mapper_amd/csrc/ltm_kernels_common.h b/lt-mapper_amd/csrc/ltm_kernels_common.h
--- a/lt-mapper_amd/csrc/ltm_kernels_common.h
+++ b/lt-mapper_amd/csrc/ltm_kernels_common.h
@@ -40,6 +40,14 @@
     bool steep_clamps;
     bool packable;
 };
+__host__ __device__ inline void group_quotient_magic(uint32_t n_groups, uint32_t& magic, uint32_t& shift)
+{
+    const uint32_t d = n_groups ? n_groups : 1u;
+    uint32_t s = 0;
+    while (((uint64_t)1 << s) < d) ++s;
+    shift = s;
+    magic = (uint32_t)((((uint64_t)1 << (26u + s)) / d) + 1u);
+}
 __host__ __device__ inline ProjLaunch make_proj_launch(Geom gg, const HostMat34& b2l, int b2l_identity, size_t M)
 {
     ProjLaunch pl;
@@ -60,11 +68,7 @@
     const size_t per_block = (size_t)kBlock * 16;
     pl.n_tiles = (uint32_t)((M + per_block - 1) / per_block);
     pl.n_tg = (pl.n_tiles + 7u) >> 3;
-    const uint32_t d = pl.n_tg ? pl.n_tg : 1u;
-    uint32_t s = 0;
-    while (((uint64_t)1 << s) < d) ++s;
-    pl.tg_shift = s;
-    pl.tg_magic = (uint32_t)((((uint64_t)1 << (26u + s)) / d) + 1u);
+    group_quotient_magic(pl.n_tg, pl.tg_magic, pl.tg_shift);
     return pl;
 }
 
@@ -86,6 +90,36 @@
     const size_t n_tg = (n_tiles + 7) / 8, n_kg = (nb + kKfPerTile - 1) / kKfPerTile;
     return (unsigned)(n_tg * 8 * kKfPerTile * n_kg);
 }
+
+static constexpr uint32_t kMaxTileRun = 16;
+struct RunLaunch {
+    uint32_t T;
+    uint32_t n_runs, n_rg;
+    uint32_t rg_magic, rg_shift;
+};
+__host__ __device__ inline RunLaunch make_run_launch(uint32_t n_tiles, uint32_t T)
+{
+    RunLaunch rl;
+    rl.T = T < 1u ? 1u : (T > kMaxTileRun ? kMaxTileRun : T);
+    rl.n_runs = n_tiles / rl.T + (n_tiles % rl.T ? 1u : 0u);
+    rl.n_rg = (rl.n_runs + 7u) >> 3;
+    group_quotient_magic(rl.n_rg, rl.rg_magic, rl.rg_shift);
+    return rl;
+}
+struct RunKf { uint32_t run, kfb; bool valid; };
+__host__ __device__ inline RunKf run_kf_of_block(uint32_t b, const RunLaunch& rl, uint32_t nb)
+{
+    static_assert(kKfPerTile == 8, "the shifts below are log2(8 XCDs) + log2(kKfPerTile)");
+    const uint32_t x = b & 7u, kfl = (b >> 3) & (kKfPerTile - 1u), q = b >> 6;
+    const uint32_t kg = (uint32_t)(((uint64_t)(b & ~63u) * rl.rg_magic) >> 32) >> rl.rg_shift;
+    const uint32_t rg = q - kg * rl.n_rg;
+    RunKf t;
+    t.run = rg * 8u + x;
+    t.kfb = kg * kKfPerTile + kfl;
+    t.valid = (t.run < rl.n_runs) & (t.kfb < nb);
+    return t;
+}
+static inline unsigned run_kf_grid(const RunLaunch& rl, size_t nb) { return tile_kf_grid(rl.n_runs, nb); }
 
 inline unsigned grid_for(size_t n, int block = kBlock)
 {
```

Result: faster. 3284 keyframe-pairs/s, median of 6 (+1.1%).
